# LuletterSoul/RP-Style-Transfer

Measured on NVIDIA B200. Metric: stylized images/sec @512^2 (multiscale RP-AdaIN transform), higher is better.
Workload: dtype f32

## Files before the change

### rp-style-transfer_b200/csrc/api.cu

```cuda
#include "common.cuh"
#include "tuning.cuh"

#include <string.h>

namespace rpst {

static thread_local char g_err[512] = "";

void set_error(const char* fmt, ...) {
    va_list ap;
    va_start(ap, fmt);
    vsnprintf(g_err, sizeof(g_err), fmt, ap);
    va_end(ap);
}

int cuda_fail(cudaError_t e, const char* what) {
    set_error("CUDA error %d (%s) in %s", (int)e, cudaGetErrorString(e), what);
    return RPST_ERR_CUDA;
}

int sm_count() {
    static int cached[64] = {0};
    int dev = 0;
    if (cudaGetDevice(&dev) != cudaSuccess || dev < 0 || dev >= 64) return 148;
    if (cached[dev] == 0) {
        int n = 0;
        if (cudaDeviceGetAttribute(&n, cudaDevAttrMultiProcessorCount, dev) != cudaSuccess || n <= 0) n = 148;
        cached[dev] = n;
    }
    return cached[dev];
}

Knobs g_knobs;

struct KnobSpec {
    const char* name;
    int64_t Knobs::*field;
    int64_t lo, hi;
};

static const KnobSpec kKnobs[] = {
    {"adain_lag_bytes", &Knobs::adain_lag_bytes, 0, INT64_MAX},
    {"adain_big_lag_bytes", &Knobs::adain_big_lag_bytes, 0, INT64_MAX},
    {"adain_mvn_lag_bytes", &Knobs::adain_mvn_lag_bytes, 0, INT64_MAX},
    {"adain_hints", &Knobs::adain_hints, 0, 1},
    {"adain_path", &Knobs::adain_path, 0, 1},
    {"adain_twin_apply", &Knobs::adain_twin_apply, 0, 1},
    {"adain_group_merge_min_spp", &Knobs::adain_group_merge_min_spp, 0, INT64_MAX},
    {"adain_merge_lead", &Knobs::adain_merge_lead, 0, INT64_MAX},
    {"seg_lag_bytes", &Knobs::seg_lag_bytes, 0, INT64_MAX},
    {"attn_flash", &Knobs::attn_flash, 0, 1},
    {"attn_flash_prof", &Knobs::attn_flash_prof, 0, INT64_MAX},
    {"wct_fused_cov", &Knobs::wct_fused_cov, 0, 1},
    {"wct_fused_apply", &Knobs::wct_fused_apply, 0, 1},
    {"wct_cov_tma", &Knobs::wct_cov_tma, 0, 1},
    {"wct_cov_prof", &Knobs::wct_cov_prof, 0, INT64_MAX},
    {"wct_roots_ns", &Knobs::wct_roots_ns, 0, 2},
    {"ns_dmma", &Knobs::ns_dmma, 0, 1},
    {"pw_x_tma", &Knobs::pw_x_tma, 0, 1},
};

static const KnobSpec* find_knob(const char* name) {
    for (const KnobSpec& k : kKnobs)
        if (!strcmp(name, k.name)) return &k;
    return nullptr;
}

int set_watchdog_adain(unsigned long long ns);
int set_watchdog_cov(unsigned long long ns);
int set_watchdog_flash(unsigned long long ns);
int set_watchdog_gemm(unsigned long long ns);
int set_watchdog_sanet(unsigned long long ns);
int set_watchdog_seg(unsigned long long ns);
int set_watchdog_pwconv(unsigned long long ns);

static int64_t g_watchdog_ms = 4000;

static int apply_watchdog(int64_t ms) {
    const unsigned long long ns = ms <= 0 ? 0ull : (unsigned long long)ms * 1000000ull;
    int count = 0, cur = 0;
    g_watchdog_ms = ms <= 0 ? 0 : ms;
    if (cudaGetDeviceCount(&count) != cudaSuccess || count <= 0) return RPST_OK;
    cudaGetDevice(&cur);
    int rc = 0;
    for (int d = 0; d < count; ++d) {
        if (cudaSetDevice(d) != cudaSuccess) continue;
        rc |= set_watchdog_adain(ns);
        rc |= set_watchdog_cov(ns);
        rc |= set_watchdog_flash(ns);
        rc |= set_watchdog_gemm(ns);
        rc |= set_watchdog_sanet(ns);
        rc |= set_watchdog_seg(ns);
        rc |= set_watchdog_pwconv(ns);
    }
    cudaSetDevice(cur);
    if (rc) {
        set_error("watchdog_ms: cudaMemcpyToSymbol failed");
        return RPST_ERR_CUDA;
    }
    return RPST_OK;
}

}

extern "C" int rpst_version(void) { return RPST_VERSION; }

namespace rpst { int64_t ns_flagged_total(); }

extern "C" const char* rpst_last_error(void) { return rpst::g_err; }

extern "C" int rpst_set_tuning(const char* name, int64_t value) {
    RPST_CHECK_ARG(name, "rpst_set_tuning: null knob name");
    if (!strcmp(name, "watchdog_ms")) return rpst::apply_watchdog(value);
    RPST_CHECK_ARG(strcmp(name, "wct_ns_flagged") != 0, "tuning knob 'wct_ns_flagged' is read-only");
    const rpst::KnobSpec* k = rpst::find_knob(name);
    RPST_CHECK_ARG(k, "unknown tuning knob '%s'", name);
    RPST_CHECK_ARG(value >= k->lo && value <= k->hi, "tuning knob '%s' takes %lld..%lld (got %lld)", name,
                   (long long)k->lo, (long long)k->hi, (long long)value);
    rpst::g_knobs.*k->field = value;
    return RPST_OK;
}

extern "C" int64_t rpst_get_tuning(const char* name) {
    if (!name) return -1;
    if (!strcmp(name, "watchdog_ms")) return rpst::g_watchdog_ms;
    if (!strcmp(name, "wct_ns_flagged")) return rpst::ns_flagged_total();
    const rpst::KnobSpec* k = rpst::find_knob(name);
    return k ? rpst::g_knobs.*k->field : -1;
}
```

### rp-style-transfer_b200/csrc/seg.cu

```cuda
#include "common.cuh"
#include "tuning.cuh"
#include "plane_io.cuh"
#include "async.cuh"

namespace rpst {
namespace {

constexpr int kLabels = 256;
constexpr int kNoIndex = 0x7f7f7f7f;

struct SegParams {
    const float* content;
    const float* style;
    const uint8_t* c_lab;
    const uint8_t* s_lab;
    const float* prev;
    float* out;
    const int* cmap;
    const int* smap;
    int64_t n, channels, hw_c, hw_s, out_batch_stride;
    float eps;
    int hints;
    int ipp_c, ipp_s, lag;
    unsigned total_items;
    unsigned* ticket;
    int* done;
    int* ready;
    int* cnt;
    int* first;
    float2* gsum;
    float4* coef;
    const int* run_flag;
};

__global__ void __launch_bounds__(256) seg_hist_kernel(const uint8_t* __restrict__ c_lab, const uint8_t* __restrict__ s_lab,
                                                       int64_t hw_c, int64_t hw_s, int* __restrict__ cnt,
                                                       int* __restrict__ first) {
    __shared__ int h[kLabels];
    __shared__ int f[kLabels];
    const int which = blockIdx.z;
    const int64_t n = blockIdx.y;
    const int64_t hw = which ? hw_s : hw_c;
    const uint8_t* lab = (which ? s_lab : c_lab) + n * hw;
    h[threadIdx.x] = 0;
    f[threadIdx.x] = kNoIndex;
    __syncthreads();
    const int64_t per_block = (hw + gridDim.x - 1) / gridDim.x;
    const int64_t beg = blockIdx.x * per_block;
    const int64_t end = beg + per_block < hw ? beg + per_block : hw;
    for (int64_t i = beg + threadIdx.x; i < end; i += blockDim.x) {
        int l = lab[i];
        atomicAdd(&h[l], 1);
        atomicMin(&f[l], (int)i);
    }
    __syncthreads();
    const int64_t slot = (n * 2 + which) * kLabels + threadIdx.x;
    if (h[threadIdx.x]) {
        atomicAdd(&cnt[slot], h[threadIdx.x]);
        atomicMin(&first[slot], f[threadIdx.x]);
    }
}

__device__ __forceinline__ int64_t src_plane(const int* map, int64_t plane) {
    return map ? (int64_t)__ldg(map + plane) : plane;
}

__device__ __forceinline__ bool label_usable(int nc, int ns) {
    return nc > 10 && ns > 10 && (int64_t)nc < 100ll * ns && (int64_t)ns < 100ll * nc;
}

struct SegItem {
    int kind;
    int64_t plane;
    int chunk;
};

__device__ __forceinline__ SegItem seg_decode(unsigned t, const SegParams& p) {
    const int64_t planes = p.n * p.channels;
    const int64_t st = p.ipp_c + p.ipp_s;
    const int64_t lag = p.lag < planes ? p.lag : planes;
    SegItem it;
    int64_t tt = t;
    auto stats = [&](int64_t plane, int64_t u) {
        it.plane = plane;
        if (u < p.ipp_c) { it.kind = 0; it.chunk = (int)u; }
        else { it.kind = 1; it.chunk = (int)(u - p.ipp_c); }
    };
    if (tt < lag * st) { stats(tt / st, tt % st); return it; }
    tt -= lag * st;
    const int64_t round = st + p.ipp_c;
    const int64_t steady = (planes - lag) * round;
    if (tt < steady) {
        int64_t r = tt / round, u = tt % round;
        if (u < st) stats(r + lag, u);
        else { it.kind = 2; it.plane = r; it.chunk = (int)(u - st); }
        return it;
    }
    tt -= steady;
    it.kind = 2; it.plane = (planes - lag) + tt / p.ipp_c; it.chunk = (int)(tt % p.ipp_c);
    return it;
}

template <int VEC>
__device__ __forceinline__ void load_labels(int (&lab)[VEC], const uint8_t* p) {
    if constexpr (VEC == 4) {
        uchar4 v = __ldg(reinterpret_cast<const uchar4*>(p));
        lab[0] = v.x; lab[1] = v.y; lab[2] = v.z; lab[3] = v.w;
    } else {
        lab[0] = __ldg(p);
    }
}

template <int VEC>
__global__ void __launch_bounds__(kPipeThreads, 3) seg_pipe_kernel(SegParams p) {
    constexpr int T = kPipeThreads;
    constexpr int CHUNK = T * kPerThread * VEC;
    static_assert(T == kLabels, "one thread per label value");
    __shared__ float s_shift[kLabels];
    __shared__ float s_acc[kLabels][2];
    __shared__ float4 s_coef[kLabels];
    __shared__ unsigned char s_use[kLabels];
    __shared__ unsigned s_ticket;
    __shared__ int s_last;

    const uint64_t pol_first = policy_evict_first();
    const uint64_t pol_last = policy_evict_last();
    const bool hint = p.hints != 0;
    const int lane = threadIdx.x & 31;
    if (p.run_flag != nullptr && __ldg(p.run_flag) == 0) return;

    if (threadIdx.x == 0) s_ticket = atomicAdd(p.ticket, 1u);
    __syncthreads();
    unsigned t = s_ticket;

    while (t < p.total_items) {
        unsigned next = 0;
        if (threadIdx.x == 0) next = atomicAdd(p.ticket, 1u);
        const SegItem it = seg_decode(t, p);
        const int64_t sample = it.plane / p.channels;
        const int* cnt_c = p.cnt + (sample * 2 + 0) * kLabels;
        const int* cnt_s = p.cnt + (sample * 2 + 1) * kLabels;

        if (it.kind < 2) {
            const bool is_style = it.kind == 1;
            const int64_t hw = is_style ? p.hw_s : p.hw_c;
            const float* x = is_style ? p.style + src_plane(p.smap, it.plane) * hw : p.content + src_plane(p.cmap, it.plane) * hw;
            const uint8_t* labels = (is_style ? p.s_lab : p.c_lab) + sample * hw;
            const int* first = p.first + (sample * 2 + it.kind) * kLabels;
            const int64_t e0 = (int64_t)it.chunk * CHUNK;
            const int64_t rem = hw - e0;
            const int nvec = (int)((rem < CHUNK ? rem : CHUNK) / VEC);
            {
                const int l = threadIdx.x;
                const bool use = label_usable(__ldg(cnt_c + l), __ldg(cnt_s + l));
                s_use[l] = use;
                s_shift[l] = use ? __ldg(x + __ldg(first + l)) : 0.f;
                s_acc[l][0] = 0.f;
                s_acc[l][1] = 0.f;
            }
            __syncthreads();
            int cur = -1;
            float shift = 0.f, a1 = 0.f, a2 = 0.f;
            const uint64_t xpol = is_style ? pol_first : pol_last;
#pragma unroll
            for (int b = 0; b < kBatches; ++b) {
                float v[kBatch][VEC];
                load_batch<VEC, T>(v, x + e0, b, nvec, xpol, hint);
#pragma unroll
                for (int j = 0; j < kBatch; ++j) {
                    const int idx = (b * kBatch + j) * T + threadIdx.x;
                    if (idx < nvec) {
                        int lab[VEC];
                        load_labels<VEC>(lab, labels + e0 + (int64_t)idx * VEC);
#pragma unroll
                        for (int e = 0; e < VEC; ++e) {
                            const int l = lab[e];
                            if (l != cur) {
                                if (cur >= 0) {
                                    atomicAdd(&s_acc[cur][0], a1);
                                    atomicAdd(&s_acc[cur][1], a2);
                                }
                                if (s_use[l]) { cur = l; shift = s_shift[l]; }
                                else cur = -1;
                                a1 = 0.f; a2 = 0.f;
                            }
                            if (cur >= 0) {
                                const float d = v[j][e] - shift;
                                a1 += d;
                                a2 = fmaf(d, d, a2);
                            }
                        }
                    }
                }
            }
            unsigned remaining = __ballot_sync(0xffffffffu, cur >= 0);
            while (remaining) {
                const int leader = __ffs(remaining) - 1;
                const int l = __shfl_sync(0xffffffffu, cur, leader);
                const bool mine = cur == l;
                const float r1 = warp_sum(mine ? a1 : 0.f);
                const float r2 = warp_sum(mine ? a2 : 0.f);
                if (lane == leader) {
                    atomicAdd(&s_acc[l][0], r1);
                    atomicAdd(&s_acc[l][1], r2);
                }
                remaining &= ~__ballot_sync(0xffffffffu, mine);
            }
            __syncthreads();
            {
                const int l = threadIdx.x;
                const float r1 = s_acc[l][0], r2 = s_acc[l][1];
                if (r1 != 0.f || r2 != 0.f) {
                    float2* g = p.gsum + (it.plane * 2 + it.kind) * kLabels + l;
                    atomicAdd(&g->x, r1);
                    atomicAdd(&g->y, r2);
                }
            }
            __threadfence();
            __syncthreads();
            if (threadIdx.x == 0) {
                int old = atomicAdd(&p.done[it.plane], 1);
                s_last = (old == p.ipp_c + p.ipp_s - 1);
            }
            __syncthreads();
            if (s_last) {
                __threadfence();
                const int l = threadIdx.x;
                const int nc = __ldg(cnt_c + l), ns = __ldg(cnt_s + l);
                float4 cf = make_float4(0.f, 1.f, 0.f, 0.f);
                if (label_usable(nc, ns)) {
                    const float kc = __ldg(p.content + src_plane(p.cmap, it.plane) * p.hw_c + __ldg(p.first + (sample * 2 + 0) * kLabels + l));
                    const float ks = __ldg(p.style + src_plane(p.smap, it.plane) * p.hw_s + __ldg(p.first + (sample * 2 + 1) * kLabels + l));
                    const float2 gc = __ldcg(p.gsum + (it.plane * 2 + 0) * kLabels + l);
                    const float2 gs = __ldcg(p.gsum + (it.plane * 2 + 1) * kLabels + l);
                    const float fnc = (float)nc, fns = (float)ns;
                    const float mu_c = kc + gc.x / fnc;
                    const float mu_s = ks + gs.x / fns;
                    const float m2c = fmaxf(gc.y - gc.x * gc.x / fnc, 0.f);
                    const float m2s = fmaxf(gs.y - gs.x * gs.x / fns, 0.f);
                    const float sd_c = sqrtf(m2c / (fnc - 1.f) + p.eps);
                    const float sd_s = sqrtf(m2s / (fns - 1.f) + p.eps);
                    cf = make_float4(mu_c, sd_s / sd_c, mu_s, 1.f);
                }
                __stcg(&p.coef[it.plane * kLabels + l], cf);
                __threadfence();
                __syncthreads();
                if (threadIdx.x == 0) st_release(&p.ready[it.plane], 1);
            }
        } else {
            const int64_t e0 = (int64_t)it.chunk * CHUNK;
            const int64_t rem = p.hw_c - e0;
            const int nvec = (int)((rem < CHUNK ? rem : CHUNK) / VEC);
            const float* cbase = p.content + src_plane(p.cmap, it.plane) * p.hw_c + e0;
            const float* pbase = p.prev ? p.prev + it.plane * p.hw_c + e0 : nullptr;
            float* obase = p.out + sample * p.out_batch_stride + (it.plane - sample * p.channels) * p.hw_c + e0;
            const uint8_t* labels = p.c_lab + sample * p.hw_c + e0;
            float c[kBatch][VEC], pv[kBatch][VEC];
            load_batch<VEC, T>(c, cbase, 0, nvec, pol_first, hint);
            if (pbase) load_batch<VEC, T>(pv, pbase, 0, nvec, pol_first, hint);
            if (threadIdx.x == 0) {
                while (ld_acquire(&p.ready[it.plane]) == 0) __nanosleep(100);
            }
            __syncthreads();
            s_coef[threadIdx.x] = __ldcg(&p.coef[it.plane * kLabels + threadIdx.x]);
            __syncthreads();
#pragma unroll
            for (int b = 0; b < kBatches; ++b) {
                if (b > 0) {
                    load_batch<VEC, T>(c, cbase, b, nvec, pol_first, hint);
                    if (pbase) load_batch<VEC, T>(pv, pbase, b, nvec, pol_first, hint);
                }
#pragma unroll
                for (int j = 0; j < kBatch; ++j) {
                    const int idx = (b * kBatch + j) * T + threadIdx.x;
                    if (idx < nvec) {
                        int lab[VEC];
                        load_labels<VEC>(lab, labels + (int64_t)idx * VEC);
                        float o[VEC];
#pragma unroll
                        for (int e = 0; e < VEC; ++e) {
                            const float4 cf = s_coef[lab[e]];
                            const float y = fmaf(c[j][e] - cf.x, cf.y, cf.z);
                            o[e] = pbase ? y + pv[j][e] : y;
                        }
                        store_vec<VEC>(obase + (int64_t)idx * VEC, o, pol_first, hint);
                    }
                }
            }
        }
        __syncthreads();
        if (threadIdx.x == 0) s_ticket = next;
        __syncthreads();
        t = s_ticket;
    }
}

constexpr int kSegItemElems = 4096;
constexpr int kSegPrevElems = 2048;
constexpr int kSegHalfElems = kSegPrevElems;
constexpr int kSegDataBytes = (kSegItemElems > 2 * kSegPrevElems ? kSegItemElems : 2 * kSegPrevElems) * 4;
constexpr int kSegStageBytes = kSegDataBytes + kSegItemElems;
constexpr int kSegDepth = 2;
constexpr int kSegGroups = 4;
constexpr int kSegGroupWarps = 4;
constexpr int kSegGroupThreads = kSegGroupWarps * 32;
constexpr int kSegWarpVecs = kSegItemElems / 4 / kSegGroupWarps;
constexpr int kSegLaneVecs = kSegWarpVecs / 32;
constexpr int kSegTicketBatch = 8;
constexpr int kMaxDense = 64;

struct SegTmaParams {
    const float* content;
    const float* style;
    const uint8_t* c_lab;
    const uint8_t* s_lab;
    const float* prev;
    float* out;
    const int* cmap;
    const int* smap;
    int64_t n, channels, hw_c, hw_s, out_batch_stride;
    float eps;
    int ic, is, lag;
    int ia, apply_elems;
    unsigned total_items;
    unsigned* ticket;
    int* ready;
    const int* cnt;
    const int* first;
    float* shift;
    const unsigned char* dense;
    const unsigned char* label_of;
    const int* dense_count;
    const int* overflow;
    float2* slots;
    int imax;
    float4* coef;
};

struct __align__(16) SegDesc {
    int64_t plane;
    int kind;
    int chunk;
    int nvec;
    int pad;
};

struct SegDecoded {
    int64_t plane;
    int kind, chunk;
};

__global__ void __launch_bounds__(kLabels) seg_dense_kernel(const int* __restrict__ cnt, unsigned char* __restrict__ dense,
                                                            unsigned char* __restrict__ label_of,
                                                            int* __restrict__ dense_count, int* __restrict__ overflow) {
    __shared__ int warp_cnt[kLabels / 32];
    const int sample = blockIdx.x, l = threadIdx.x, lane = l & 31, w = l >> 5;
    const bool use = label_usable(cnt[(sample * 2 + 0) * kLabels + l], cnt[(sample * 2 + 1) * kLabels + l]);
    const unsigned m = __ballot_sync(0xffffffffu, use);
    if (lane == 0) warp_cnt[w] = __popc(m);
    __syncthreads();
    int base = 0, total = 0;
    for (int i = 0; i < kLabels / 32; ++i) {
        if (i < w) base += warp_cnt[i];
        total += warp_cnt[i];
    }
    const int id = base + __popc(m & ((1u << lane) - 1u));
    dense[sample * kLabels + l] = (use && id < kMaxDense) ? (unsigned char)id : (unsigned char)255;
    if (use && id < kMaxDense) label_of[sample * kMaxDense + id] = (unsigned char)l;
    if (l == 0) {
        dense_count[sample] = total < kMaxDense ? total : kMaxDense;
        if (total > kMaxDense) atomicOr(overflow, 1);
    }
}

__global__ void seg_shift_kernel(SegTmaParams p) {
    const int64_t planes = p.n * p.channels;
    const int64_t idx = blockIdx.x * (int64_t)blockDim.x + threadIdx.x;
    if (idx >= planes * 2 * kLabels) return;
    const int l = (int)(idx % kLabels), which = (int)((idx / kLabels) & 1);
    const int64_t plane = idx / (2 * kLabels), sample = plane / p.channels;
    const int slot = (int)((sample * 2 + which) * kLabels + l);
    float v = 0.f;
    if (p.cnt[slot] > 0) {
        v = which ? p.style[src_plane(p.smap, plane) * p.hw_s + p.first[slot]]
                  : p.content[src_plane(p.cmap, plane) * p.hw_c + p.first[slot]];
    }
    p.shift[idx] = v;
}

__device__ __forceinline__ bool slot2_valid(double2 v) {
    return (unsigned)(__double_as_longlong(v.x) >> 32) != 0xffffffffu && (unsigned)(__double_as_longlong(v.y) >> 32) != 0xffffffffu;
}
__device__ __forceinline__ double2 ld_slot2(const double2* p) {
    double2 v;
    asm volatile("ld.global.cg.v2.f64 {%0,%1}, [%2];" : "=d"(v.x), "=d"(v.y) : "l"(p) : "memory");
    return v;
}
__device__ __forceinline__ float2 ld_slot1(const float2* p) {
    float2 v;
    asm volatile("ld.global.cg.v2.f32 {%0,%1}, [%2];" : "=f"(v.x), "=f"(v.y) : "l"(p) : "memory");
    return v;
}
__device__ __forceinline__ bool slot1_valid(float2 v) {
    return __float_as_uint(v.x) != 0xffffffffu && __float_as_uint(v.y) != 0xffffffffu;
}

__device__ __forceinline__ float canon_f(float v) {
    return __float_as_uint(v) == 0xffffffffu ? __uint_as_float(0x7fc00000u) : v;
}

__device__ __forceinline__ void seg_decode(unsigned t, const SegTmaParams& p, int& kind, int64_t& plane, int& chunk) {
    const unsigned P = (unsigned)(p.n * p.channels), L = (unsigned)p.lag, Lm = L - 1;
    const unsigned Ic = (unsigned)p.ic, St = (unsigned)(p.ic + p.is), Ia = (unsigned)p.ia;
    auto stat = [&](unsigned pl, unsigned u) {
        plane = pl;
        if (u < Ic) { kind = 0; chunk = (int)u; } else { kind = 1; chunk = (int)(u - Ic); }
    };
    unsigned n = (L - Lm) * St;
    if (t < n) { stat(t / St, t % St); return; }
    t -= n; n = Lm * (St + 1);
    if (t < n) {
        const unsigned j = t / (St + 1), u = t % (St + 1);
        if (u < St) stat((L - Lm) + j, u); else { kind = 3; plane = j; chunk = 0; }
        return;
    }
    t -= n; n = (P - L) * (St + 1 + Ia);
    if (t < n) {
        const unsigned j = t / (St + 1 + Ia), u = t % (St + 1 + Ia);
        if (u < St) stat(L + j, u);
        else if (u == St) { kind = 3; plane = Lm + j; chunk = 0; }
        else { kind = 2; plane = j; chunk = (int)(u - St - 1); }
        return;
    }
    t -= n; n = (L - Lm) * (1 + Ia);
    if (t < n) {
        const unsigned j = t / (1 + Ia), u = t % (1 + Ia);
        if (u == 0) { kind = 3; plane = (P - L + Lm) + j; chunk = 0; }
        else { kind = 2; plane = (P - L) + j; chunk = (int)(u - 1); }
        return;
    }
    t -= n;
    kind = 2; plane = (P - Lm) + t / Ia; chunk = (int)(t % Ia);
}

constexpr int kSegCoefBytes = (kMaxDense + 2) * 16;
constexpr int kSegCacheBytes = (kSegCoefBytes + kLabels * 4 + kLabels + 2 * kMaxDense * 2 * 4 +
                                kSegGroupWarps * 32 * 16 + 2 * kSegGroupWarps * 32 * 2 * 4 + 127) / 128 * 128;
constexpr int kSegMergeThreads = 64;
constexpr int kSegMailbox = 8;

__device__ __forceinline__ void seg_warp_totals(float2* tab, int lane, int cur, float a1, float a2) {
    const int key = cur >= 0 ? cur : -1;
    const unsigned peers = __match_any_sync(0xffffffffu, key);
    const int steps = (int)__reduce_max_sync(0xffffffffu, (unsigned)__popc(peers));
    float s1 = a1, s2 = a2;
    unsigned rem = peers & (peers - 1u);
    const bool leader = (peers & ((1u << lane) - 1u)) == 0u;
    for (int k = 1; k < steps; ++k) {
        const int src = rem ? __ffs(rem) - 1 : lane;
        const float x1 = __shfl_sync(0xffffffffu, a1, src), x2 = __shfl_sync(0xffffffffu, a2, src);
        if (rem) { s1 += x1; s2 += x2; }
        rem &= rem - 1u;
    }
    tab[lane] = make_float2(0.f, 0.f);
    __syncwarp();
    if (leader && key >= 0) tab[key] = make_float2(s1, s2);
    __syncwarp();
}

__global__ void __launch_bounds__(32 + kSegGroups * kSegGroupThreads + kSegMergeThreads, 1) seg_tma_kernel(SegTmaParams p) {
    constexpr int S = kSegGroups * kSegDepth;
    constexpr int STAGE_BYTES = kSegStageBytes;
    constexpr int CACHE_BYTES = kSegCacheBytes;
    extern __shared__ __align__(128) unsigned char smem_raw[];
    unsigned char* stages = smem_raw;
    unsigned char* caches = smem_raw + (size_t)S * STAGE_BYTES;
    SegDesc* desc = reinterpret_cast<SegDesc*>(caches + (size_t)kSegGroups * ((CACHE_BYTES + 127) / 128 * 128));
    uint64_t* full = reinterpret_cast<uint64_t*>(desc + S);
    uint64_t* empty = full + S;
    uint64_t* mfull = empty + S;
    uint64_t* mempty = mfull + kSegMailbox;
    int64_t* mbox = reinterpret_cast<int64_t*>(mempty + kSegMailbox);
    SegDecoded* dec = reinterpret_cast<SegDecoded*>(mbox + kSegMailbox);

    const int warp = threadIdx.x >> 5, lane = threadIdx.x & 31;
    if (__ldg(p.overflow) != 0) return;
    if (threadIdx.x == 0) {
        for (int s = 0; s < S; ++s) {
            mbar_init(&full[s], 1);
            mbar_init(&empty[s], kSegGroupWarps);
        }
        for (int s = 0; s < kSegMailbox; ++s) {
            mbar_init(&mfull[s], 1);
            mbar_init(&mempty[s], kSegMergeThreads / 32);
        }
        mbar_fence_init();
    }
    __syncthreads();

    if (warp == 0) {
        const uint64_t pol_first = policy_evict_first();
        const uint64_t pol_last = policy_evict_last();
        unsigned next_base = 0;
        if (lane == 0) next_base = atomicAdd(p.ticket, (unsigned)kSegTicketBatch) + 1u;
        unsigned seq = 0, mseq = 0;
        for (;;) {
            const unsigned base = __shfl_sync(0xffffffffu, next_base, 0);
            if (lane == 0) next_base = atomicAdd(p.ticket, (unsigned)kSegTicketBatch) + 1u;
            static_assert(kSegGroups * kSegDepth >= kSegTicketBatch, "a batch must not reuse a stage");
            int kind = 3, chunk = 0;
            int64_t plane = 0, splane = 0;
            if (lane < kSegTicketBatch) {
                kind = -1;
                const unsigned t = base + (unsigned)lane;
                if (t < p.total_items) seg_decode(t, p, kind, plane, chunk);
                dec[lane].kind = kind; dec[lane].chunk = chunk; dec[lane].plane = plane;
                if (kind == 1) splane = src_plane(p.smap, plane);
                else if (kind == 0 || kind == 2) splane = src_plane(p.cmap, plane);
            }
            __syncwarp();
            const unsigned stopmask = __ballot_sync(0xffffffffu, kind < 0);
            const int nvalid = stopmask ? __ffs(stopmask) - 1 : kSegTicketBatch;
            if (lane == 0) {
                for (int i = 0; i < nvalid; ++i) {
                    if (dec[i].kind == 3) {
                        const int ms = (int)(mseq % kSegMailbox);
                        mbar_wait_quiet(&mempty[ms], ((mseq / kSegMailbox) & 1u) ^ 1u);
                        mbox[ms] = dec[i].plane;
                        mbar_arrive(&mfull[ms]);
                        ++mseq;
                    }
                }
            }
            const bool is_item = lane < nvalid && kind != 3;
            const unsigned itemmask = __ballot_sync(0xffffffffu, is_item);
            const int my_pos = __popc(itemmask & ((1u << lane) - 1u));
            if (is_item) {
                const unsigned my_seq = seq + (unsigned)my_pos;
                const unsigned k = my_seq / kSegGroups;
                const int stage = (int)(my_seq % kSegGroups) * kSegDepth + (int)(k % kSegDepth);
                mbar_wait_quiet(&empty[stage], ((k / kSegDepth) & 1u) ^ 1u);
                SegDesc* d = &desc[stage];
                d->plane = plane; d->kind = kind; d->chunk = chunk;
                const bool is_style = kind == 1;
                const int64_t hw = is_style ? p.hw_s : p.hw_c;
                const int item_elems = kind == 2 ? p.apply_elems : kSegItemElems;
                const int64_t e0 = (int64_t)chunk * item_elems;
                const int64_t rem = hw - e0;
                const int nvec = (int)((rem < item_elems ? rem : item_elems) / 4);
                d->nvec = nvec;
                const uint32_t bytes = (uint32_t)nvec * 16u;
                unsigned char* st = stages + (size_t)stage * STAGE_BYTES;
                const int64_t sample = (int)plane / (int)p.channels;
                const float* src = (is_style ? p.style : p.content) + splane * hw + e0;
                const uint8_t* lab = (is_style ? p.s_lab : p.c_lab) + sample * hw + e0;
                const bool has_prev = kind == 2 && p.prev != nullptr;
                mbar_arrive_expect_tx(&full[stage], bytes + (has_prev ? bytes : 0u) + (uint32_t)nvec * 4u);
                tma_load_1d(st, src, bytes, &full[stage], kind == 0 ? pol_last : pol_first);
                if (has_prev)
                    tma_load_1d(st + kSegHalfElems * 4, p.prev + plane * hw + e0, bytes, &full[stage], pol_first);
                tma_load_1d(st + kSegDataBytes, lab, (uint32_t)nvec * 4u, &full[stage], pol_last);
            }
            __syncwarp();
            seq += (unsigned)__popc(itemmask);
            bool finished = false;
            if (stopmask != 0u) {
                if (lane == 0) {
                    for (int g = 0; g < kSegGroups; ++g, ++seq) {
                        const unsigned k = seq / kSegGroups;
                        const int stage = (int)(seq % kSegGroups) * kSegDepth + (int)(k % kSegDepth);
                        mbar_wait_quiet(&empty[stage], ((k / kSegDepth) & 1u) ^ 1u);
                        desc[stage].kind = -1;
                        mbar_arrive(&full[stage]);
                    }
                    const int ms = (int)(mseq % kSegMailbox);
                    mbar_wait_quiet(&mempty[ms], ((mseq / kSegMailbox) & 1u) ^ 1u);
                    mbox[ms] = -1;
                    mbar_arrive(&mfull[ms]);
                }
                finished = true;
            }
            if (finished) return;
            __syncwarp();
        }
    }

    if (warp > kSegGroups * kSegGroupWarps) {
        __shared__ double s_merge[kSegMergeThreads][4];
        const int t = threadIdx.x - (32 + kSegGroups * kSegGroupThreads);
        for (unsigned mseq = 0;; ++mseq) {
            const int ms = (int)(mseq % kSegMailbox);
            mbar_wait_quiet(&mfull[ms], (mseq / kSegMailbox) & 1u, 64);
            const int64_t plane = mbox[ms];
            __syncwarp();
            if (lane == 0) mbar_arrive(&mempty[ms]);
            if (plane < 0) break;
            const int64_t sample = plane / p.channels;
            const int dcount = __ldg(p.dense_count + sample);
            const int parts = dcount > 0 ? kSegMergeThreads / dcount : 1;
            const int dn = dcount > 0 ? t % dcount : 0;
            const int part = dcount > 0 ? t / dcount : parts;
            double s4[4] = {0.0, 0.0, 0.0, 0.0};
            if (part < parts) {
#pragma unroll
                for (int which = 0; which < 2; ++which) {
                    const int items = which ? p.is : p.ic;
                    const int per = (items + parts - 1) / parts;
                    const int lo = part * per, hi = min(items, lo + per);
                    const float2* base = p.slots + ((plane * 2 + which) * p.imax) * kMaxDense + dn;
                    constexpr int kUnroll = 32;
                    for (int c0 = lo; c0 < hi; c0 += kUnroll) {
                        float2 v[kUnroll];
#pragma unroll
                        for (int u = 0; u < kUnroll; ++u) {
                            v[u] = make_float2(0.f, 0.f);
                            if (c0 + u < hi) v[u] = ld_slot1(base + (int64_t)(c0 + u) * kMaxDense);
                        }
#pragma unroll
                        for (int u = 0; u < kUnroll; ++u) {
                            if (c0 + u < hi) {
                                if (!slot1_valid(v[u])) {
                                    const float2* sp = base + (int64_t)(c0 + u) * kMaxDense;
                                    const uint64_t t0 = global_timer_ns();
                                    do {
                                        __nanosleep(64);
                                        v[u] = ld_slot1(sp);
                                        if (watchdog_expired(t0)) __trap();
                                    } while (!slot1_valid(v[u]));
                                }
                                s4[which * 2 + 0] += (double)v[u].x;
                                s4[which * 2 + 1] += (double)v[u].y;
                            }
                        }
                    }
                }
            }
#pragma unroll
            for (int q = 0; q < 4; ++q) s_merge[t][q] = s4[q];
            named_bar_sync(15, kSegMergeThreads);
            if (t < dcount) {
                for (int q = 1; q < parts; ++q) {
#pragma unroll
                    for (int e = 0; e < 4; ++e) s4[e] += s_merge[q * dcount + t][e];
                }
                const int l = __ldg(p.label_of + sample * kMaxDense + dn);
                const double dnc = (double)__ldg(p.cnt + (sample * 2 + 0) * kLabels + l);
                const double dns = (double)__ldg(p.cnt + (sample * 2 + 1) * kLabels + l);
                const double kc = (double)__ldg(p.shift + (plane * 2 + 0) * kLabels + l);
                const double ks = (double)__ldg(p.shift + (plane * 2 + 1) * kLabels + l);
                const double mu_c = kc + s4[0] / dnc, mu_s = ks + s4[2] / dns;
                const double m2c = fmax(s4[1] - s4[0] * s4[0] / dnc, 0.0), m2s = fmax(s4[3] - s4[2] * s4[2] / dns, 0.0);
                const double sd_c = sqrt(m2c / (dnc - 1.0) + (double)p.eps), sd_s = sqrt(m2s / (dns - 1.0) + (double)p.eps);
                __stcg(&p.coef[plane * kLabels + l], make_float4((float)mu_c, (float)(sd_s / sd_c), (float)mu_s, 1.f));
            }
            for (int l = t; l < kLabels; l += kSegMergeThreads)
                if (__ldg(p.dense + sample * kLabels + l) == 255) __stcg(&p.coef[plane * kLabels + l], make_float4(0.f, 1.f, 0.f, 0.f));
            __threadfence();
            named_bar_sync(15, kSegMergeThreads);
            if (t == 0) st_release(&p.ready[plane], 1);
        }
        return;
    }

    const int group = (warp - 1) / kSegGroupWarps;
    const int gw = (warp - 1) % kSegGroupWarps;
    const int gt = gw * 32 + lane;
    unsigned char* cache = caches + (size_t)group * ((CACHE_BYTES + 127) / 128 * 128);
    float4* c_coef = reinterpret_cast<float4*>(cache);
    float* c_shift = reinterpret_cast<float*>(cache + kSegCoefBytes);
    unsigned char* c_dense = cache + kSegCoefBytes + kLabels * 4;
    float* c_acc = reinterpret_cast<float*>(c_dense + kLabels);
    float4* c_stage = reinterpret_cast<float4*>(c_acc + 2 * kMaxDense * 2);
    float* c_wtot = reinterpret_cast<float*>(c_stage + kSegGroupWarps * 32);
    const uint64_t pol_first = policy_evict_first();
    int64_t cached_stat = -1;
    int64_t cached_apply = -1;
    int64_t cached_sample = -1;
    int dcount = 0;
    unsigned sparity = 0;
    for (int i = gt; i < 2 * kMaxDense * 2; i += kSegGroupThreads) c_acc[i] = 0.f;
    named_bar_sync(1 + group, kSegGroupThreads);

    for (unsigned seq = group;; seq += kSegGroups) {
        const unsigned k = seq / kSegGroups;
        const int stage = group * kSegDepth + (int)(k % kSegDepth);
        mbar_wait_quiet(&full[stage], (k / kSegDepth) & 1u);
        const SegDesc* d = &desc[stage];
        const int kind = d->kind;
        if (kind < 0) break;
        const int64_t plane = d->plane;
        const int chunk = d->chunk;
        const int warp_vecs = (kind == 2 ? p.apply_elems : kSegItemElems) / 4 / kSegGroupWarps;
        const int wvec = min(max(d->nvec - gw * warp_vecs, 0), warp_vecs);
        const int64_t sample = (int)plane / (int)p.channels;
        unsigned char* st = stages + (size_t)stage * STAGE_BYTES;
        const float4* a4 = reinterpret_cast<const float4*>(st) + gw * warp_vecs;
        const float4* b4 = reinterpret_cast<const float4*>(st + kSegHalfElems * 4) + gw * warp_vecs;
        const uint32_t* l4 = reinterpret_cast<const uint32_t*>(st + kSegDataBytes) + gw * warp_vecs;

        {
            if (sample != cached_sample) {
                named_bar_sync(1 + group, kSegGroupThreads);
                for (int l = gt; l < kLabels; l += kSegGroupThreads) c_dense[l] = __ldg(p.dense + sample * kLabels + l);
                dcount = __ldg(p.dense_count + sample);
                named_bar_sync(1 + group, kSegGroupThreads);
                cached_sample = sample;
            }
        }

        if (kind <= 1) {
            const int64_t key = plane * 2 + kind;
            if (key != cached_stat) {
                named_bar_sync(1 + group, kSegGroupThreads);
                for (int l = gt; l < kLabels; l += kSegGroupThreads) c_shift[l] = __ldg(p.shift + key * kLabels + l);
                named_bar_sync(1 + group, kSegGroupThreads);
                cached_stat = key;
            }
            float* acc = c_acc + sparity * (kMaxDense * 2);
            int cur = -1;
            uint32_t cur4 = 0xffffffffu;
            float shift = 0.f, a1 = 0.f, a2 = 0.f;
            float4 vv[kSegLaneVecs];
            uint32_t lww[kSegLaneVecs];
#pragma unroll
            for (int j = 0; j < kSegLaneVecs; ++j) {
                const int idx = lane * kSegLaneVecs + ((j + lane) & (kSegLaneVecs - 1));
                if (idx < wvec) { vv[j] = a4[idx]; lww[j] = l4[idx]; }
            }
            __syncwarp();
            if (lane == 0) mbar_arrive(&empty[stage]);
#pragma unroll
            for (int j = 0; j < kSegLaneVecs; ++j) {
                const int idx = lane * kSegLaneVecs + ((j + lane) & (kSegLaneVecs - 1));
                if (idx < wvec) {
                    const float4 v = vv[j];
                    const uint32_t lw = lww[j];
                    if (lw == cur4 && cur >= 0) {
                        const float d0 = v.x - shift, d1 = v.y - shift, d2 = v.z - shift, d3 = v.w - shift;
                        a1 += (d0 + d1) + (d2 + d3);
                        a2 = fmaf(d0, d0, a2); a2 = fmaf(d1, d1, a2); a2 = fmaf(d2, d2, a2); a2 = fmaf(d3, d3, a2);
                    } else {
                        const float e[4] = {v.x, v.y, v.z, v.w};
                        int curl = cur >= 0 ? (int)(cur4 & 0xffu) : -1;
#pragma unroll
                        for (int q = 0; q < 4; ++q) {
                            const int l = (int)((lw >> (8 * q)) & 0xffu);
                            if (l != curl) {
                                if (cur >= 0) {
                                    atomicAdd(&acc[cur * 2 + 0], a1);
                                    atomicAdd(&acc[cur * 2 + 1], a2);
                                }
                                const int dn = c_dense[l];
                                curl = l;
                                if (dn != 255) { cur = dn; shift = c_shift[l]; cur4 = (uint32_t)l * 0x01010101u; }
                                else { cur = -1; cur4 = 0xffffffffu; }
                                a1 = 0.f; a2 = 0.f;
                            }
                            if (cur >= 0) {
                                const float dd = e[q] - shift;
                                a1 += dd;
                                a2 = fmaf(dd, dd, a2);
                            }
                        }
                    }
                }
            }
            const bool staged = dcount <= 32;
            float* wt = c_wtot + (sparity * kSegGroupWarps + gw) * 64;
            if (staged) {
                seg_warp_totals(reinterpret_cast<float2*>(wt), lane, cur, a1, a2);
            } else if (cur >= 0) {
                atomicAdd(&acc[cur * 2 + 0], a1);
                atomicAdd(&acc[cur * 2 + 1], a2);
            }
            named_bar_sync(1 + group, kSegGroupThreads);
            if (gt < dcount) {
                float t1 = acc[gt * 2 + 0], t2 = acc[gt * 2 + 1];
                if (staged) {
                    const float* w0 = c_wtot + sparity * kSegGroupWarps * 64;
#pragma unroll
                    for (int q = 0; q < kSegGroupWarps; ++q) { t1 += w0[q * 64 + gt * 2 + 0]; t2 += w0[q * 64 + gt * 2 + 1]; }
                }
                const float s1 = canon_f(t1), s2 = canon_f(t2);
                acc[gt * 2 + 0] = 0.f;
                acc[gt * 2 + 1] = 0.f;
                float2* slot = p.slots + ((key * p.imax + chunk) * kMaxDense + gt);
                asm volatile("st.global.cg.v2.f32 [%0], {%1,%2};" :: "l"(slot), "f"(s1), "f"(s2) : "memory");
            }
            sparity ^= 1u;
        } else if (kind == 2) {
            if (plane != cached_apply) {
                if (lane == 0 && ld_acquire(&p.ready[plane]) == 0) {
                    const uint64_t t0 = global_timer_ns();
                    while (ld_acquire(&p.ready[plane]) == 0) {
                        __nanosleep(64);
                        if (watchdog_expired(t0)) __trap();
                    }
                }
                named_bar_sync(1 + group, kSegGroupThreads);
                if (gt < dcount) c_coef[gt] = __ldcg(&p.coef[plane * kLabels + __ldg(p.label_of + sample * kMaxDense + gt)]);
                if (gt == kSegGroupThreads - 1) c_coef[kMaxDense] = make_float4(0.f, 1.f, 0.f, 0.f);
                named_bar_sync(1 + group, kSegGroupThreads);
                cached_apply = plane;
            }
            const bool has_prev = p.prev != nullptr;
            float4* o4 = reinterpret_cast<float4*>(p.out + sample * p.out_batch_stride + (plane - sample * p.channels) * p.hw_c +
                                                   (int64_t)chunk * p.apply_elems) + gw * warp_vecs;
            uint32_t last_w = 0;
            float4 cf = c_coef[kMaxDense];
            bool have = false;
            auto coef_of = [&](uint32_t l) -> float4 { const int dn = c_dense[l]; return c_coef[dn < kMaxDense ? dn : kMaxDense]; };
#pragma unroll 8
            for (int j = 0; j < kSegLaneVecs; ++j) {
                const int idx = j * 32 + lane;
                if (idx < wvec) {
                    const float4 v = a4[idx];
                    const uint32_t lw = l4[idx];
                    float4 o;
                    const uint32_t b0 = lw & 0xffu;
                    if (lw == b0 * 0x01010101u) {
                        if (!have || lw != last_w) { cf = coef_of(b0); last_w = lw; have = true; }
                        o.x = fmaf(v.x - cf.x, cf.y, cf.z);
                        o.y = fmaf(v.y - cf.x, cf.y, cf.z);
                        o.z = fmaf(v.z - cf.x, cf.y, cf.z);
                        o.w = fmaf(v.w - cf.x, cf.y, cf.z);
                    } else {
                        const float4 c0 = coef_of(b0), c1 = coef_of((lw >> 8) & 0xffu), c2 = coef_of((lw >> 16) & 0xffu),
                                     c3 = coef_of(lw >> 24);
                        o.x = fmaf(v.x - c0.x, c0.y, c0.z);
                        o.y = fmaf(v.y - c1.x, c1.y, c1.z);
                        o.z = fmaf(v.z - c2.x, c2.y, c2.z);
                        o.w = fmaf(v.w - c3.x, c3.y, c3.z);
                    }
                    if (has_prev) {
                        const float4 q = b4[idx];
                        o.x += q.x; o.y += q.y; o.z += q.z; o.w += q.w;
                    }
                    stg_f4_hint(reinterpret_cast<float*>(o4 + idx), o, pol_first);
                }
            }
            __syncwarp();
            if (lane == 0) mbar_arrive(&empty[stage]);
        }
    }
}

__global__ void seg_export_info_kernel(const int* __restrict__ cnt, int32_t* __restrict__ info, int64_t n) {
    const int64_t i = blockIdx.x * (int64_t)blockDim.x + threadIdx.x;
    if (i >= n * kLabels) return;
    const int64_t s = i / kLabels, l = i % kLabels;
    const int nc = cnt[(s * 2 + 0) * kLabels + l], ns = cnt[(s * 2 + 1) * kLabels + l];
    info[i * 3 + 0] = nc;
    info[i * 3 + 1] = ns;
    info[i * 3 + 2] = label_usable(nc, ns) ? 1 : 0;
}

struct SegLayout {
    size_t zero_bytes;
    size_t first_off, first_bytes, coef_off, total;
    size_t done_off, cnt_off, gsum_off;
};

SegLayout seg_layout(int64_t n, int64_t c) {
    const size_t planes = (size_t)(n * c);
    SegLayout l;
    l.done_off = 256;
    l.cnt_off = align_up(l.done_off + planes * 2 * sizeof(int), 256);
    l.gsum_off = align_up(l.cnt_off + (size_t)n * 2 * kLabels * sizeof(int), 256);
    l.zero_bytes = align_up(l.gsum_off + planes * 2 * kLabels * sizeof(float2), 256);
    l.first_off = l.zero_bytes;
    l.first_bytes = align_up((size_t)n * 2 * kLabels * sizeof(int), 256);
    l.coef_off = l.first_off + l.first_bytes;
    l.total = align_up(l.coef_off + planes * kLabels * sizeof(float4), 256);
    return l;
}

inline bool aligned(const void* p, size_t a) { return (reinterpret_cast<uintptr_t>(p) & (a - 1)) == 0; }

struct SegTmaLayout {
    size_t ticket, zero_beg, ready, cnt, dcount, overflow, zero_end, first, first_bytes, shift, dense, label_of, coef,
        slots, slots_bytes, total;
};
SegTmaLayout seg_tma_layout(int64_t n, int64_t c, int64_t hw_c, int64_t hw_s) {
    const size_t planes = (size_t)(n * c);
    const size_t ic = (size_t)((hw_c + kSegItemElems - 1) / kSegItemElems), is = (size_t)((hw_s + kSegItemElems - 1) / kSegItemElems);
    const size_t imax = ic > is ? ic : is;
    SegTmaLayout l;
    size_t o = 0;
    auto take = [&](size_t bytes) { size_t at = o; o += align_up(bytes, 256); return at; };
    l.ticket = take(256);
    l.zero_beg = o;
    l.ready = take(planes * sizeof(int));
    l.cnt = take((size_t)n * 2 * kLabels * sizeof(int));
    l.dcount = take((size_t)n * sizeof(int));
    l.overflow = take(sizeof(int));
    l.zero_end = o;
    l.first_bytes = align_up((size_t)n * 2 * kLabels * sizeof(int), 256);
    l.first = take(l.first_bytes);
    l.shift = take(planes * 2 * kLabels * sizeof(float));
    l.dense = take((size_t)n * kLabels);
    l.label_of = take((size_t)n * kMaxDense);
    l.coef = take(planes * kLabels * sizeof(float4));
    l.slots_bytes = planes * 2 * imax * kMaxDense * sizeof(float2);
    l.slots = take(l.slots_bytes);
    l.total = o;
    return l;
}

int launch_seg_tma(const SegTmaParams& p, cudaStream_t st) {
    constexpr size_t stage = kSegStageBytes;
    constexpr size_t cache = kSegCacheBytes;
    constexpr size_t smem = kSegGroups * (kSegDepth * stage + cache) + kSegGroups * kSegDepth * sizeof(SegDesc) +
                            2 * kSegGroups * kSegDepth * sizeof(uint64_t) + 2 * kSegMailbox * sizeof(uint64_t) +
                            kSegMailbox * sizeof(int64_t) +
                            kSegTicketBatch * sizeof(SegDecoded);
    static PerDeviceFlag configured_on;
    bool& configured = configured_on.get();
    if (!configured) {
        RPST_CUDA(cudaFuncSetAttribute(seg_tma_kernel, cudaFuncAttributeMaxDynamicSharedMemorySize, (int)smem));
        configured = true;
    }
    int64_t grid = sm_count();
    if (grid > (int64_t)p.total_items) grid = p.total_items;
    seg_tma_kernel<<<(int)grid, 32 + kSegGroups * kSegGroupThreads + kSegMergeThreads, smem, st>>>(p);
    RPST_CUDA(cudaGetLastError());
    return RPST_OK;
}

}
}

namespace rpst {
namespace {
int64_t seg_plan_schedule(SegTmaParams& q, bool has_prev) {
    const int64_t planes = q.n * q.channels;
    q.ic = (int)((q.hw_c + kSegItemElems - 1) / kSegItemElems);
    q.is = (int)((q.hw_s + kSegItemElems - 1) / kSegItemElems);
    q.imax = q.ic > q.is ? q.ic : q.is;
    q.apply_elems = has_prev ? kSegPrevElems : kSegItemElems;
    q.ia = (int)((q.hw_c + q.apply_elems - 1) / q.apply_elems);
    const int64_t plane_bytes = q.hw_c * (int64_t)sizeof(float);
    int64_t lag = (g_knobs.seg_lag_bytes + plane_bytes - 1) / plane_bytes;
    if (lag < 3) lag = 3;
    q.lag = (int)(lag < planes ? lag : planes);
    return planes * ((int64_t)q.ic + q.is + 1 + q.ia);
}

__global__ void seg_schedule_dump_kernel(SegTmaParams p, int32_t* out) {
    const unsigned t = blockIdx.x * blockDim.x + threadIdx.x;
    if (t >= p.total_items) return;
    int kind = -1, chunk = 0;
    int64_t plane = 0;
    seg_decode(t, p, kind, plane, chunk);
    out[3 * (size_t)t + 0] = kind;
    out[3 * (size_t)t + 1] = (int32_t)plane;
    out[3 * (size_t)t + 2] = chunk;
}
}
}

using namespace rpst;

#ifdef RPST_DEBUG_EXPORTS
extern "C" int rpst_debug_seg_schedule(int64_t n, int64_t c, int64_t hw_c, int64_t hw_s, int has_prev, int32_t* tickets,
                                       int64_t max_tickets, int64_t* info, void* stream) {
    RPST_CHECK_ARG(n > 0 && c > 0 && hw_c > 0 && hw_s > 0 && info != nullptr, "debug_seg_schedule: bad arguments");
    SegTmaParams q{};
    q.n = n; q.channels = c; q.hw_c = hw_c; q.hw_s = hw_s;
    const int64_t total = seg_plan_schedule(q, has_prev != 0);
    RPST_CHECK_ARG(total < (1ll << 31), "debug_seg_schedule: too many tickets");
    q.total_items = (unsigned)total;
    info[0] = total; info[1] = q.ic; info[2] = q.is; info[3] = q.ia; info[4] = q.lag;
    if (tickets != nullptr) {
        RPST_CHECK_ARG(max_tickets >= total, "debug_seg_schedule: ticket buffer too small");
        seg_schedule_dump_kernel<<<(unsigned)((total + 255) / 256), 256, 0, static_cast<cudaStream_t>(stream)>>>(q, tickets);
        RPST_CUDA(cudaGetLastError());
    }
    return RPST_OK;
}
#endif

extern "C" size_t rpst_seg_adain_workspace_bytes(int64_t n, int64_t c, int64_t hw_c, int64_t hw_s) {
    if (n <= 0 || c <= 0) return 256;
    return seg_layout(n, c).total + seg_tma_layout(n, c, hw_c, hw_s).total;

}

namespace {
int seg_adain_fwd_impl(const float* content, const float* style, const uint8_t* c_labels, const uint8_t* s_labels,
                       const float* prev, float* out, int64_t n, int64_t c, int64_t hw_c, int64_t hw_s,
                       int64_t out_batch_stride, float eps, const int* content_map, const int* style_map,
                       int32_t* label_info, void* workspace, size_t workspace_bytes, void* stream);
}

extern "C" int rpst_seg_adain_fwd(const float* content, const float* style, const uint8_t* c_labels,
                                  const uint8_t* s_labels, const float* prev, float* out, int64_t n, int64_t c,
                                  int64_t hw_c, int64_t hw_s, float eps, int32_t* label_info, void* workspace,
                                  size_t workspace_bytes, void* stream) {
    return seg_adain_fwd_impl(content, style, c_labels, s_labels, prev, out, n, c, hw_c, hw_s, c * hw_c, eps, nullptr,
                              nullptr, label_info, workspace, workspace_bytes, stream);
}

extern "C" int rpst_seg_adain_fwd_mapped(const float* content, const float* style, const uint8_t* c_labels,
                                         const uint8_t* s_labels, const float* prev, float* out, int64_t n, int64_t c,
                                         int64_t hw_c, int64_t hw_s, int64_t out_batch_stride, float eps,
                                         const int32_t* content_map, const int32_t* style_map, int32_t* label_info,
                                         void* workspace, size_t workspace_bytes, void* stream) {
    RPST_CHECK_ARG(n * c < (1ll << 31), "seg_adain_mapped: plane index does not fit int32");
    return seg_adain_fwd_impl(content, style, c_labels, s_labels, prev, out, n, c, hw_c, hw_s, out_batch_stride, eps,
                              content_map, style_map, label_info, workspace, workspace_bytes, stream);
}

namespace {
int seg_adain_fwd_impl(const float* content, const float* style, const uint8_t* c_labels, const uint8_t* s_labels,
                       const float* prev, float* out, int64_t n, int64_t c, int64_t hw_c, int64_t hw_s,
                       int64_t out_batch_stride, float eps, const int* content_map, const int* style_map,
                       int32_t* label_info, void* workspace, size_t workspace_bytes, void* stream) {
    RPST_CHECK_ARG(n >= 0 && c >= 0 && hw_c >= 0 && hw_s >= 0, "seg_adain: negative size");
    if (n == 0 || c == 0 || hw_c == 0) return RPST_OK;
    RPST_CHECK_ARG(content && style && c_labels && s_labels && out, "seg_adain: null pointer");
    RPST_CHECK_ARG(hw_s > 0, "seg_adain: empty style map");
    RPST_CHECK_ARG(hw_c < (1ll << 31) && hw_s < (1ll << 31), "seg_adain: plane too large");
    RPST_CHECK_ARG(out_batch_stride >= c * hw_c, "seg_adain: out_batch_stride (%lld) < c*hw_c (%lld)",
                   (long long)out_batch_stride, (long long)(c * hw_c));
    RPST_CHECK_ARG(out != content && out != style && out != prev, "seg_adain: out must not alias an input");
    const size_t need = rpst_seg_adain_workspace_bytes(n, c, hw_c, hw_s);
    if (workspace == nullptr || workspace_bytes < need) {
        set_error("seg_adain: workspace too small (%zu < %zu bytes)", workspace_bytes, need);
        return RPST_ERR_WORKSPACE;
    }
    RPST_CHECK_ARG(aligned(workspace, 256), "seg_adain: workspace must be 256-byte aligned");
    cudaStream_t st = static_cast<cudaStream_t>(stream);
    char* base = static_cast<char*>(workspace);
    const int64_t hw_max0 = hw_c > hw_s ? hw_c : hw_s;
    int hist_blocks0 = (int)((hw_max0 + 16383) / 16384);
    if (hist_blocks0 > 256) hist_blocks0 = 256;
    const bool tma_ok = g_knobs.adain_path == 0 && hw_c % 16 == 0 && hw_s % 16 == 0 &&
                        aligned(content, 16) && aligned(style, 16) && aligned(out, 16) && out_batch_stride % 4 == 0 &&
                        (!prev || aligned(prev, 16)) && aligned(c_labels, 16) && aligned(s_labels, 16);
    const int* run_flag = nullptr;
    if (tma_ok) {
        const SegTmaLayout t = seg_tma_layout(n, c, hw_c, hw_s);
        SegTmaParams q{};
        q.content = content; q.style = style; q.c_lab = c_labels; q.s_lab = s_labels; q.prev = prev; q.out = out;
        q.cmap = content_map; q.smap = style_map;
        q.n = n; q.channels = c; q.hw_c = hw_c; q.hw_s = hw_s; q.out_batch_stride = out_batch_stride; q.eps = eps;
        q.ticket = reinterpret_cast<unsigned*>(base + t.ticket);
        q.ready = reinterpret_cast<int*>(base + t.ready);
        int* cnt = reinterpret_cast<int*>(base + t.cnt);
        int* first = reinterpret_cast<int*>(base + t.first);
        int* dcount = reinterpret_cast<int*>(base + t.dcount);
        int* overflow = reinterpret_cast<int*>(base + t.overflow);
        unsigned char* dense = reinterpret_cast<unsigned char*>(base + t.dense);
        unsigned char* label_of = reinterpret_cast<unsigned char*>(base + t.label_of);
        q.cnt = cnt; q.first = first; q.dense = dense; q.label_of = label_of; q.dense_count = dcount; q.overflow = overflow;
        q.shift = reinterpret_cast<float*>(base + t.shift);
        q.coef = reinterpret_cast<float4*>(base + t.coef);
        q.slots = reinterpret_cast<float2*>(base + t.slots);
        RPST_CUDA(cudaMemsetAsync(base + t.ticket, 0xff, 256, st));
        RPST_CUDA(cudaMemsetAsync(base + t.zero_beg, 0, t.zero_end - t.zero_beg, st));
        RPST_CUDA(cudaMemsetAsync(base + t.first, 0x7f, t.first_bytes, st));
        RPST_CUDA(cudaMemsetAsync(base + t.slots, 0xff, t.slots_bytes, st));
        seg_hist_kernel<<<dim3(hist_blocks0, (unsigned)n, 2), 256, 0, st>>>(c_labels, s_labels, hw_c, hw_s, cnt, first);
        RPST_CUDA(cudaGetLastError());
        seg_dense_kernel<<<(unsigned)n, kLabels, 0, st>>>(cnt, dense, label_of, dcount, overflow);
        RPST_CUDA(cudaGetLastError());
        if (label_info) {
            const int64_t tot = n * kLabels;
            seg_export_info_kernel<<<(unsigned)((tot + 255) / 256), 256, 0, st>>>(cnt, label_info, n);
            RPST_CUDA(cudaGetLastError());
            label_info = nullptr;
        }
        const int64_t planes = n * c;
        seg_shift_kernel<<<(unsigned)((planes * 2 * kLabels + 255) / 256), 256, 0, st>>>(q);
        RPST_CUDA(cudaGetLastError());
        const int64_t total = seg_plan_schedule(q, prev != nullptr);
        RPST_CHECK_ARG(total < (1ll << 31), "seg_adain: too many work items (%lld); split the call", (long long)total);
        q.total_items = (unsigned)total;
        const int rc = launch_seg_tma(q, st);
        if (rc) return rc;
        run_flag = overflow;
        base += t.total;
    }
    const SegLayout l = seg_layout(n, c);
    SegParams p{};
    p.content = content; p.style = style; p.c_lab = c_labels; p.s_lab = s_labels; p.prev = prev; p.out = out;
    p.cmap = content_map; p.smap = style_map;
    p.n = n; p.channels = c; p.hw_c = hw_c; p.hw_s = hw_s; p.out_batch_stride = out_batch_stride; p.eps = eps;
    p.hints = (int)g_knobs.adain_hints;
    p.ticket = reinterpret_cast<unsigned*>(base);
    p.done = reinterpret_cast<int*>(base + l.done_off);
    p.ready = p.done + n * c;
    p.cnt = reinterpret_cast<int*>(base + l.cnt_off);
    p.gsum = reinterpret_cast<float2*>(base + l.gsum_off);
    p.first = reinterpret_cast<int*>(base + l.first_off);
    p.coef = reinterpret_cast<float4*>(base + l.coef_off);
    p.run_flag = run_flag;
    RPST_CUDA(cudaMemsetAsync(base, 0, l.zero_bytes, st));
    RPST_CUDA(cudaMemsetAsync(base + l.first_off, 0x7f, l.first_bytes, st));

    const int64_t hw_max = hw_c > hw_s ? hw_c : hw_s;
    int hist_blocks = (int)((hw_max + 16383) / 16384);
    if (hist_blocks > 256) hist_blocks = 256;
    seg_hist_kernel<<<dim3(hist_blocks, (unsigned)n, 2), 256, 0, st>>>(c_labels, s_labels, hw_c, hw_s, p.cnt, p.first);
    RPST_CUDA(cudaGetLastError());
    if (label_info) {
        const int64_t tot = n * kLabels;
        seg_export_info_kernel<<<(unsigned)((tot + 255) / 256), 256, 0, st>>>(p.cnt, label_info, n);
        RPST_CUDA(cudaGetLastError());
    }

    const bool vec = hw_c % 4 == 0 && hw_s % 4 == 0 && aligned(content, 16) && aligned(style, 16) && aligned(out, 16) &&
                     out_batch_stride % 4 == 0 && (!prev || aligned(prev, 16)) && aligned(c_labels, 4) && aligned(s_labels, 4);
    const int64_t chunk = (int64_t)kPipeThreads * kPerThread * (vec ? 4 : 1);
    p.ipp_c = (int)((hw_c + chunk - 1) / chunk);
    p.ipp_s = (int)((hw_s + chunk - 1) / chunk);
    const int64_t plane_bytes = hw_c * (int64_t)sizeof(float);
    int64_t lag = (g_knobs.adain_lag_bytes + plane_bytes - 1) / plane_bytes;
    if (lag < 3) lag = 3;
    const int64_t planes = n * c;
    p.lag = (int)(lag < planes ? lag : planes);
    const int64_t total = planes * (2ll * p.ipp_c + p.ipp_s);
    RPST_CHECK_ARG(total < (1ll << 31), "seg_adain: too many work items (%lld); split the call", (long long)total);
    p.total_items = (unsigned)total;
    int64_t grid = (int64_t)sm_count() * 3;
    if (grid > total) grid = total;
    if (vec) seg_pipe_kernel<4><<<(int)grid, kPipeThreads, 0, st>>>(p);
    else seg_pipe_kernel<1><<<(int)grid, kPipeThreads, 0, st>>>(p);
    RPST_CUDA(cudaGetLastError());
    return RPST_OK;
}
}

RPST_WATCHDOG_SETTER(seg)
```

### rp-style-transfer_b200/csrc/tuning.cuh

```cuda
#pragma once
#include <stdint.h>

namespace rpst {

struct Knobs {
    int64_t adain_lag_bytes = 32ll << 20;
    int64_t adain_big_lag_bytes = 128ll << 20;
    int64_t adain_mvn_lag_bytes = 44ll << 20;
    int64_t adain_hints = 1;
    int64_t adain_path = 0;
    int64_t adain_twin_apply = 1;
    int64_t adain_group_merge_min_spp = 512;
    int64_t adain_merge_lead = 0;
    int64_t seg_lag_bytes = 256ll << 20;
    int64_t attn_flash = 1;
    int64_t attn_flash_prof = 0;
    int64_t wct_fused_cov = 1;
    int64_t wct_fused_apply = 1;
    int64_t wct_cov_tma = 1;
    int64_t wct_cov_prof = 0;
    int64_t wct_roots_ns = 1;
    int64_t ns_dmma = 1;
    int64_t pw_x_tma = 1;
};

extern Knobs g_knobs;

}
```

Baseline: 3478.

## Split persistent segmented AdaIN kernel into stats, merge and apply launches

Replaces the single persistent warp-specialized TMA kernel, which used a ticket scheduler, lagged per-plane merge mailboxes and per-item slot buffers, with three ordinary launches: a multi-CTA stats kernel that writes per-row double partials, a per-plane merge kernel, and an apply kernel. This removes the ticket atomics, spin-waits and slot memsets, and lets more stats CTAs reside per SM. In exchange it loses the overlap between statistics and apply work, adds launch boundaries, and re-reads content planes from memory in the apply pass. The lag knob is replaced by a rows-per-CTA knob.

```diff
diff --git a/rp-style-transfer_b200/csrc/api.cu b/rp-style-transfer_b200/csrc/api.cu
--- a/rp-style-transfer_b200/csrc/api.cu
+++ b/rp-style-transfer_b200/csrc/api.cu
@@ -48,7 +48,7 @@
     {"adain_twin_apply", &Knobs::adain_twin_apply, 0, 1},
     {"adain_group_merge_min_spp", &Knobs::adain_group_merge_min_spp, 0, INT64_MAX},
     {"adain_merge_lead", &Knobs::adain_merge_lead, 0, INT64_MAX},
-    {"seg_lag_bytes", &Knobs::seg_lag_bytes, 0, INT64_MAX},
+    {"seg_stats_items", &Knobs::seg_stats_items, 1, 1024},
     {"attn_flash", &Knobs::attn_flash, 0, 1},
     {"attn_flash_prof", &Knobs::attn_flash_prof, 0, INT64_MAX},
     {"wct_fused_cov", &Knobs::wct_fused_cov, 0, 1},
diff --git a/rp-style-transfer_b200/csrc/seg.cu b/rp-style-transfer_b200/csrc/seg.cu
--- a/rp-style-transfer_b200/csrc/seg.cu
+++ b/rp-style-transfer_b200/csrc/seg.cu
@@ -297,16 +297,15 @@
 
 constexpr int kSegItemElems = 4096;
 constexpr int kSegPrevElems = 2048;
-constexpr int kSegHalfElems = kSegPrevElems;
-constexpr int kSegDataBytes = (kSegItemElems > 2 * kSegPrevElems ? kSegItemElems : 2 * kSegPrevElems) * 4;
-constexpr int kSegStageBytes = kSegDataBytes + kSegItemElems;
-constexpr int kSegDepth = 2;
-constexpr int kSegGroups = 4;
+constexpr int kSegStageBytes = kSegItemElems * 4 + kSegItemElems;
+constexpr int kSegStages = 2;
+constexpr int kSegStatsCtas = 5;
 constexpr int kSegGroupWarps = 4;
 constexpr int kSegGroupThreads = kSegGroupWarps * 32;
 constexpr int kSegWarpVecs = kSegItemElems / 4 / kSegGroupWarps;
 constexpr int kSegLaneVecs = kSegWarpVecs / 32;
-constexpr int kSegTicketBatch = 8;
+constexpr int kSegApplyThreads = 256;
+constexpr int kSegApplyChunks = 8;
 constexpr int kMaxDense = 64;
 
 struct SegTmaParams {
@@ -320,11 +319,10 @@
     const int* smap;
     int64_t n, channels, hw_c, hw_s, out_batch_stride;
     float eps;
-    int ic, is, lag;
+    int ic, is;
     int ia, apply_elems;
-    unsigned total_items;
-    unsigned* ticket;
-    int* ready;
+    int row_items;
+    int rc, rs;
     const int* cnt;
     const int* first;
     float* shift;
@@ -332,22 +330,8 @@
     const unsigned char* label_of;
     const int* dense_count;
     const int* overflow;
-    float2* slots;
-    int imax;
+    double2* rows;
     float4* coef;
-};
-
-struct __align__(16) SegDesc {
-    int64_t plane;
-    int kind;
-    int chunk;
-    int nvec;
-    int pad;
-};
-
-struct SegDecoded {
-    int64_t plane;
-    int kind, chunk;
 };
 
 __global__ void __launch_bounds__(kLabels) seg_dense_kernel(const int* __restrict__ cnt, unsigned char* __restrict__ dense,
@@ -388,67 +372,6 @@
     p.shift[idx] = v;
 }
 
-__device__ __forceinline__ bool slot2_valid(double2 v) {
-    return (unsigned)(__double_as_longlong(v.x) >> 32) != 0xffffffffu && (unsigned)(__double_as_longlong(v.y) >> 32) != 0xffffffffu;
-}
-__device__ __forceinline__ double2 ld_slot2(const double2* p) {
-    double2 v;
-    asm volatile("ld.global.cg.v2.f64 {%0,%1}, [%2];" : "=d"(v.x), "=d"(v.y) : "l"(p) : "memory");
-    return v;
-}
-__device__ __forceinline__ float2 ld_slot1(const float2* p) {
-    float2 v;
-    asm volatile("ld.global.cg.v2.f32 {%0,%1}, [%2];" : "=f"(v.x), "=f"(v.y) : "l"(p) : "memory");
-    return v;
-}
-__device__ __forceinline__ bool slot1_valid(float2 v) {
-    return __float_as_uint(v.x) != 0xffffffffu && __float_as_uint(v.y) != 0xffffffffu;
-}
-
-__device__ __forceinline__ float canon_f(float v) {
-    return __float_as_uint(v) == 0xffffffffu ? __uint_as_float(0x7fc00000u) : v;
-}
-
-__device__ __forceinline__ void seg_decode(unsigned t, const SegTmaParams& p, int& kind, int64_t& plane, int& chunk) {
-    const unsigned P = (unsigned)(p.n * p.channels), L = (unsigned)p.lag, Lm = L - 1;
-    const unsigned Ic = (unsigned)p.ic, St = (unsigned)(p.ic + p.is), Ia = (unsigned)p.ia;
-    auto stat = [&](unsigned pl, unsigned u) {
-        plane = pl;
-        if (u < Ic) { kind = 0; chunk = (int)u; } else { kind = 1; chunk = (int)(u - Ic); }
-    };
-    unsigned n = (L - Lm) * St;
-    if (t < n) { stat(t / St, t % St); return; }
-    t -= n; n = Lm * (St + 1);
-    if (t < n) {
-        const unsigned j = t / (St + 1), u = t % (St + 1);
-        if (u < St) stat((L - Lm) + j, u); else { kind = 3; plane = j; chunk = 0; }
-        return;
-    }
-    t -= n; n = (P - L) * (St + 1 + Ia);
-    if (t < n) {
-        const unsigned j = t / (St + 1 + Ia), u = t % (St + 1 + Ia);
-        if (u < St) stat(L + j, u);
-        else if (u == St) { kind = 3; plane = Lm + j; chunk = 0; }
-        else { kind = 2; plane = j; chunk = (int)(u - St - 1); }
-        return;
-    }
-    t -= n; n = (L - Lm) * (1 + Ia);
-    if (t < n) {
-        const unsigned j = t / (1 + Ia), u = t % (1 + Ia);
-        if (u == 0) { kind = 3; plane = (P - L + Lm) + j; chunk = 0; }
-        else { kind = 2; plane = (P - L) + j; chunk = (int)(u - 1); }
-        return;
-    }
-    t -= n;
-    kind = 2; plane = (P - Lm) + t / Ia; chunk = (int)(t % Ia);
-}
-
-constexpr int kSegCoefBytes = (kMaxDense + 2) * 16;
-constexpr int kSegCacheBytes = (kSegCoefBytes + kLabels * 4 + kLabels + 2 * kMaxDense * 2 * 4 +
-                                kSegGroupWarps * 32 * 16 + 2 * kSegGroupWarps * 32 * 2 * 4 + 127) / 128 * 128;
-constexpr int kSegMergeThreads = 64;
-constexpr int kSegMailbox = 8;
-
 __device__ __forceinline__ void seg_warp_totals(float2* tab, int lane, int cur, float a1, float a2) {
     const int key = cur >= 0 ? cur : -1;
     const unsigned peers = __match_any_sync(0xffffffffu, key);
@@ -468,379 +391,235 @@
     __syncwarp();
 }
 
-__global__ void __launch_bounds__(32 + kSegGroups * kSegGroupThreads + kSegMergeThreads, 1) seg_tma_kernel(SegTmaParams p) {
-    constexpr int S = kSegGroups * kSegDepth;
-    constexpr int STAGE_BYTES = kSegStageBytes;
-    constexpr int CACHE_BYTES = kSegCacheBytes;
-    extern __shared__ __align__(128) unsigned char smem_raw[];
-    unsigned char* stages = smem_raw;
-    unsigned char* caches = smem_raw + (size_t)S * STAGE_BYTES;
-    SegDesc* desc = reinterpret_cast<SegDesc*>(caches + (size_t)kSegGroups * ((CACHE_BYTES + 127) / 128 * 128));
-    uint64_t* full = reinterpret_cast<uint64_t*>(desc + S);
-    uint64_t* empty = full + S;
-    uint64_t* mfull = empty + S;
-    uint64_t* mempty = mfull + kSegMailbox;
-    int64_t* mbox = reinterpret_cast<int64_t*>(mempty + kSegMailbox);
-    SegDecoded* dec = reinterpret_cast<SegDecoded*>(mbox + kSegMailbox);
-
+template <class Release>
+__device__ __forceinline__ void seg_item_stats(const float4* a4, const uint32_t* l4, int wvec, int lane,
+                                               const unsigned char* c_dense, const float* c_shift, float* acc,
+                                               float* wt, bool staged, Release release) {
+    int cur = -1;
+    uint32_t cur4 = 0xffffffffu;
+    float shift = 0.f, a1 = 0.f, a2 = 0.f;
+    float4 vv[kSegLaneVecs];
+    uint32_t lww[kSegLaneVecs];
+#pragma unroll
+    for (int j = 0; j < kSegLaneVecs; ++j) {
+        const int idx = lane * kSegLaneVecs + ((j + lane) & (kSegLaneVecs - 1));
+        if (idx < wvec) { vv[j] = a4[idx]; lww[j] = l4[idx]; }
+    }
+#pragma unroll
+    for (int j = 0; j < kSegLaneVecs; ++j) {
+        const int idx = lane * kSegLaneVecs + ((j + lane) & (kSegLaneVecs - 1));
+        if (idx < wvec) {
+            const float4 v = vv[j];
+            const uint32_t lw = lww[j];
+            if (lw == cur4 && cur >= 0) {
+                const float d0 = v.x - shift, d1 = v.y - shift, d2 = v.z - shift, d3 = v.w - shift;
+                a1 += (d0 + d1) + (d2 + d3);
+                a2 = fmaf(d0, d0, a2); a2 = fmaf(d1, d1, a2); a2 = fmaf(d2, d2, a2); a2 = fmaf(d3, d3, a2);
+            } else {
+                const float e[4] = {v.x, v.y, v.z, v.w};
+                int curl = cur >= 0 ? (int)(cur4 & 0xffu) : -1;
+#pragma unroll
+                for (int q = 0; q < 4; ++q) {
+                    const int l = (int)((lw >> (8 * q)) & 0xffu);
+                    if (l != curl) {
+                        if (cur >= 0) {
+                            atomicAdd(&acc[cur * 2 + 0], a1);
+                            atomicAdd(&acc[cur * 2 + 1], a2);
+                        }
+                        const int dn = c_dense[l];
+                        curl = l;
+                        if (dn != 255) { cur = dn; shift = c_shift[l]; cur4 = (uint32_t)l * 0x01010101u; }
+                        else { cur = -1; cur4 = 0xffffffffu; }
+                        a1 = 0.f; a2 = 0.f;
+                    }
+                    if (cur >= 0) {
+                        const float dd = e[q] - shift;
+                        a1 += dd;
+                        a2 = fmaf(dd, dd, a2);
+                    }
+                }
+            }
+        }
+    }
+    release();
+    if (staged) {
+        seg_warp_totals(reinterpret_cast<float2*>(wt), lane, cur, a1, a2);
+    } else if (cur >= 0) {
+        atomicAdd(&acc[cur * 2 + 0], a1);
+        atomicAdd(&acc[cur * 2 + 1], a2);
+    }
+}
+
+__global__ void __launch_bounds__(32 + kSegGroupThreads, kSegStatsCtas) seg_stats_kernel(SegTmaParams p) {
+    __shared__ __align__(128) unsigned char stages[kSegStages][kSegStageBytes];
+    __shared__ uint64_t full[kSegStages], empty[kSegStages];
+    __shared__ float c_shift[kLabels];
+    __shared__ unsigned char c_dense[kLabels];
+    __shared__ float c_acc[2][kMaxDense * 2];
+    __shared__ float c_wtot[2][kSegGroupWarps * 64];
+    if (__ldg(p.overflow) != 0) return;
+
+    const int rows = p.rc + p.rs;
+    const int64_t plane = blockIdx.x / rows;
+    const int row = (int)(blockIdx.x % rows);
+    const int which = row < p.rc ? 0 : 1;
+    const int i0 = (which ? row - p.rc : row) * p.row_items;
+    const int count = min(p.row_items, (which ? p.is : p.ic) - i0);
+    const int64_t sample = plane / p.channels;
+    const int64_t hw = which ? p.hw_s : p.hw_c;
     const int warp = threadIdx.x >> 5, lane = threadIdx.x & 31;
-    if (__ldg(p.overflow) != 0) return;
     if (threadIdx.x == 0) {
-        for (int s = 0; s < S; ++s) {
+        for (int s = 0; s < kSegStages; ++s) {
             mbar_init(&full[s], 1);
             mbar_init(&empty[s], kSegGroupWarps);
         }
-        for (int s = 0; s < kSegMailbox; ++s) {
-            mbar_init(&mfull[s], 1);
-            mbar_init(&mempty[s], kSegMergeThreads / 32);
-        }
         mbar_fence_init();
     }
+    for (int l = threadIdx.x; l < kLabels; l += blockDim.x) {
+        c_shift[l] = __ldg(p.shift + (plane * 2 + which) * kLabels + l);
+        c_dense[l] = __ldg(p.dense + sample * kLabels + l);
+    }
+    for (int i = threadIdx.x; i < 2 * kMaxDense * 2; i += blockDim.x) (&c_acc[0][0])[i] = 0.f;
     __syncthreads();
 
     if (warp == 0) {
-        const uint64_t pol_first = policy_evict_first();
-        const uint64_t pol_last = policy_evict_last();
-        unsigned next_base = 0;
-        if (lane == 0) next_base = atomicAdd(p.ticket, (unsigned)kSegTicketBatch) + 1u;
-        unsigned seq = 0, mseq = 0;
-        for (;;) {
-            const unsigned base = __shfl_sync(0xffffffffu, next_base, 0);
-            if (lane == 0) next_base = atomicAdd(p.ticket, (unsigned)kSegTicketBatch) + 1u;
-            static_assert(kSegGroups * kSegDepth >= kSegTicketBatch, "a batch must not reuse a stage");
-            int kind = 3, chunk = 0;
-            int64_t plane = 0, splane = 0;
-            if (lane < kSegTicketBatch) {
-                kind = -1;
-                const unsigned t = base + (unsigned)lane;
-                if (t < p.total_items) seg_decode(t, p, kind, plane, chunk);
-                dec[lane].kind = kind; dec[lane].chunk = chunk; dec[lane].plane = plane;
-                if (kind == 1) splane = src_plane(p.smap, plane);
-                else if (kind == 0 || kind == 2) splane = src_plane(p.cmap, plane);
-            }
-            __syncwarp();
-            const unsigned stopmask = __ballot_sync(0xffffffffu, kind < 0);
-            const int nvalid = stopmask ? __ffs(stopmask) - 1 : kSegTicketBatch;
-            if (lane == 0) {
-                for (int i = 0; i < nvalid; ++i) {
-                    if (dec[i].kind == 3) {
-                        const int ms = (int)(mseq % kSegMailbox);
-                        mbar_wait_quiet(&mempty[ms], ((mseq / kSegMailbox) & 1u) ^ 1u);
-                        mbox[ms] = dec[i].plane;
-                        mbar_arrive(&mfull[ms]);
-                        ++mseq;
-                    }
-                }
-            }
-            const bool is_item = lane < nvalid && kind != 3;
-            const unsigned itemmask = __ballot_sync(0xffffffffu, is_item);
-            const int my_pos = __popc(itemmask & ((1u << lane) - 1u));
-            if (is_item) {
-                const unsigned my_seq = seq + (unsigned)my_pos;
-                const unsigned k = my_seq / kSegGroups;
-                const int stage = (int)(my_seq % kSegGroups) * kSegDepth + (int)(k % kSegDepth);
-                mbar_wait_quiet(&empty[stage], ((k / kSegDepth) & 1u) ^ 1u);
-                SegDesc* d = &desc[stage];
-                d->plane = plane; d->kind = kind; d->chunk = chunk;
-                const bool is_style = kind == 1;
-                const int64_t hw = is_style ? p.hw_s : p.hw_c;
-                const int item_elems = kind == 2 ? p.apply_elems : kSegItemElems;
-                const int64_t e0 = (int64_t)chunk * item_elems;
-                const int64_t rem = hw - e0;
-                const int nvec = (int)((rem < item_elems ? rem : item_elems) / 4);
-                d->nvec = nvec;
-                const uint32_t bytes = (uint32_t)nvec * 16u;
-                unsigned char* st = stages + (size_t)stage * STAGE_BYTES;
-                const int64_t sample = (int)plane / (int)p.channels;
-                const float* src = (is_style ? p.style : p.content) + splane * hw + e0;
-                const uint8_t* lab = (is_style ? p.s_lab : p.c_lab) + sample * hw + e0;
-                const bool has_prev = kind == 2 && p.prev != nullptr;
-                mbar_arrive_expect_tx(&full[stage], bytes + (has_prev ? bytes : 0u) + (uint32_t)nvec * 4u);
-                tma_load_1d(st, src, bytes, &full[stage], kind == 0 ? pol_last : pol_first);
-                if (has_prev)
-                    tma_load_1d(st + kSegHalfElems * 4, p.prev + plane * hw + e0, bytes, &full[stage], pol_first);
-                tma_load_1d(st + kSegDataBytes, lab, (uint32_t)nvec * 4u, &full[stage], pol_last);
-            }
-            __syncwarp();
-            seq += (unsigned)__popc(itemmask);
-            bool finished = false;
-            if (stopmask != 0u) {
-                if (lane == 0) {
-                    for (int g = 0; g < kSegGroups; ++g, ++seq) {
-                        const unsigned k = seq / kSegGroups;
-                        const int stage = (int)(seq % kSegGroups) * kSegDepth + (int)(k % kSegDepth);
-                        mbar_wait_quiet(&empty[stage], ((k / kSegDepth) & 1u) ^ 1u);
-                        desc[stage].kind = -1;
-                        mbar_arrive(&full[stage]);
-                    }
-                    const int ms = (int)(mseq % kSegMailbox);
-                    mbar_wait_quiet(&mempty[ms], ((mseq / kSegMailbox) & 1u) ^ 1u);
-                    mbox[ms] = -1;
-                    mbar_arrive(&mfull[ms]);
-                }
-                finished = true;
-            }
-            if (finished) return;
-            __syncwarp();
-        }
-    }
-
-    if (warp > kSegGroups * kSegGroupWarps) {
-        __shared__ double s_merge[kSegMergeThreads][4];
-        const int t = threadIdx.x - (32 + kSegGroups * kSegGroupThreads);
-        for (unsigned mseq = 0;; ++mseq) {
-            const int ms = (int)(mseq % kSegMailbox);
-            mbar_wait_quiet(&mfull[ms], (mseq / kSegMailbox) & 1u, 64);
-            const int64_t plane = mbox[ms];
-            __syncwarp();
-            if (lane == 0) mbar_arrive(&mempty[ms]);
-            if (plane < 0) break;
-            const int64_t sample = plane / p.channels;
-            const int dcount = __ldg(p.dense_count + sample);
-            const int parts = dcount > 0 ? kSegMergeThreads / dcount : 1;
-            const int dn = dcount > 0 ? t % dcount : 0;
-            const int part = dcount > 0 ? t / dcount : parts;
-            double s4[4] = {0.0, 0.0, 0.0, 0.0};
-            if (part < parts) {
-#pragma unroll
-                for (int which = 0; which < 2; ++which) {
-                    const int items = which ? p.is : p.ic;
-                    const int per = (items + parts - 1) / parts;
-                    const int lo = part * per, hi = min(items, lo + per);
-                    const float2* base = p.slots + ((plane * 2 + which) * p.imax) * kMaxDense + dn;
-                    constexpr int kUnroll = 32;
-                    for (int c0 = lo; c0 < hi; c0 += kUnroll) {
-                        float2 v[kUnroll];
-#pragma unroll
-                        for (int u = 0; u < kUnroll; ++u) {
-                            v[u] = make_float2(0.f, 0.f);
-                            if (c0 + u < hi) v[u] = ld_slot1(base + (int64_t)(c0 + u) * kMaxDense);
-                        }
-#pragma unroll
-                        for (int u = 0; u < kUnroll; ++u) {
-                            if (c0 + u < hi) {
-                                if (!slot1_valid(v[u])) {
-                                    const float2* sp = base + (int64_t)(c0 + u) * kMaxDense;
-                                    const uint64_t t0 = global_timer_ns();
-                                    do {
-                                        __nanosleep(64);
-                                        v[u] = ld_slot1(sp);
-                                        if (watchdog_expired(t0)) __trap();
-                                    } while (!slot1_valid(v[u]));
-                                }
-                                s4[which * 2 + 0] += (double)v[u].x;
-                                s4[which * 2 + 1] += (double)v[u].y;
-                            }
-                        }
-                    }
-                }
-            }
-#pragma unroll
-            for (int q = 0; q < 4; ++q) s_merge[t][q] = s4[q];
-            named_bar_sync(15, kSegMergeThreads);
-            if (t < dcount) {
-                for (int q = 1; q < parts; ++q) {
-#pragma unroll
-                    for (int e = 0; e < 4; ++e) s4[e] += s_merge[q * dcount + t][e];
-                }
-                const int l = __ldg(p.label_of + sample * kMaxDense + dn);
-                const double dnc = (double)__ldg(p.cnt + (sample * 2 + 0) * kLabels + l);
-                const double dns = (double)__ldg(p.cnt + (sample * 2 + 1) * kLabels + l);
-                const double kc = (double)__ldg(p.shift + (plane * 2 + 0) * kLabels + l);
-                const double ks = (double)__ldg(p.shift + (plane * 2 + 1) * kLabels + l);
-                const double mu_c = kc + s4[0] / dnc, mu_s = ks + s4[2] / dns;
-                const double m2c = fmax(s4[1] - s4[0] * s4[0] / dnc, 0.0), m2s = fmax(s4[3] - s4[2] * s4[2] / dns, 0.0);
-                const double sd_c = sqrt(m2c / (dnc - 1.0) + (double)p.eps), sd_s = sqrt(m2s / (dns - 1.0) + (double)p.eps);
-                __stcg(&p.coef[plane * kLabels + l], make_float4((float)mu_c, (float)(sd_s / sd_c), (float)mu_s, 1.f));
-            }
-            for (int l = t; l < kLabels; l += kSegMergeThreads)
-                if (__ldg(p.dense + sample * kLabels + l) == 255) __stcg(&p.coef[plane * kLabels + l], make_float4(0.f, 1.f, 0.f, 0.f));
-            __threadfence();
-            named_bar_sync(15, kSegMergeThreads);
-            if (t == 0) st_release(&p.ready[plane], 1);
+        if (lane == 0) {
+            const float* src = which ? p.style + src_plane(p.smap, plane) * hw : p.content + src_plane(p.cmap, plane) * hw;
+            const uint8_t* lab = (which ? p.s_lab : p.c_lab) + sample * hw;
+            const uint64_t pol_first = policy_evict_first();
+            const uint64_t pol_last = policy_evict_last();
+            for (int k = 0; k < count; ++k) {
+                const int s = k % kSegStages;
+                mbar_wait_quiet(&empty[s], ((k / kSegStages) & 1u) ^ 1u);
+                fence_proxy_async_smem();
+                const int64_t e0 = (int64_t)(i0 + k) * kSegItemElems;
+                const uint32_t elems = (uint32_t)min(hw - e0, (int64_t)kSegItemElems);
+                mbar_arrive_expect_tx(&full[s], elems * 5u);
+                tma_load_1d(stages[s], src + e0, elems * 4u, &full[s], pol_first);
+                tma_load_1d(stages[s] + kSegItemElems * 4, lab + e0, elems, &full[s], pol_last);
+            }
         }
         return;
     }
 
-    const int group = (warp - 1) / kSegGroupWarps;
-    const int gw = (warp - 1) % kSegGroupWarps;
-    const int gt = gw * 32 + lane;
-    unsigned char* cache = caches + (size_t)group * ((CACHE_BYTES + 127) / 128 * 128);
-    float4* c_coef = reinterpret_cast<float4*>(cache);
-    float* c_shift = reinterpret_cast<float*>(cache + kSegCoefBytes);
-    unsigned char* c_dense = cache + kSegCoefBytes + kLabels * 4;
-    float* c_acc = reinterpret_cast<float*>(c_dense + kLabels);
-    float4* c_stage = reinterpret_cast<float4*>(c_acc + 2 * kMaxDense * 2);
-    float* c_wtot = reinterpret_cast<float*>(c_stage + kSegGroupWarps * 32);
+    const int gw = warp - 1, gt = threadIdx.x - 32;
+    const int dcount = __ldg(p.dense_count + sample);
+    const bool staged = dcount <= 32;
+    double s1 = 0.0, s2 = 0.0;
+    for (int k = 0; k < count; ++k) {
+        const int s = k % kSegStages, par = k & 1;
+        mbar_wait_quiet(&full[s], (k / kSegStages) & 1u);
+        const int nvec = (int)(min(hw - (int64_t)(i0 + k) * kSegItemElems, (int64_t)kSegItemElems) / 4);
+        const int wvec = min(max(nvec - gw * kSegWarpVecs, 0), kSegWarpVecs);
+        const float4* a4 = reinterpret_cast<const float4*>(stages[s]) + gw * kSegWarpVecs;
+        const uint32_t* l4 = reinterpret_cast<const uint32_t*>(stages[s] + kSegItemElems * 4) + gw * kSegWarpVecs;
+        seg_item_stats(a4, l4, wvec, lane, c_dense, c_shift, c_acc[par], c_wtot[par] + gw * 64, staged, [&] {
+            __syncwarp();
+            if (lane == 0) mbar_arrive(&empty[s]);
+        });
+        named_bar_sync(1, kSegGroupThreads);
+        if (gt < dcount) {
+            float t1 = c_acc[par][gt * 2 + 0], t2 = c_acc[par][gt * 2 + 1];
+            if (staged) {
+#pragma unroll
+                for (int q = 0; q < kSegGroupWarps; ++q) { t1 += c_wtot[par][q * 64 + gt * 2 + 0]; t2 += c_wtot[par][q * 64 + gt * 2 + 1]; }
+            }
+            c_acc[par][gt * 2 + 0] = 0.f;
+            c_acc[par][gt * 2 + 1] = 0.f;
+            s1 += (double)t1;
+            s2 += (double)t2;
+        }
+    }
+    if (gt < dcount) p.rows[((int64_t)blockIdx.x * kMaxDense) + gt] = make_double2(s1, s2);
+}
+
+__global__ void seg_merge_kernel(SegTmaParams p) {
+    if (__ldg(p.overflow) != 0) return;
+    const int64_t plane = blockIdx.x, sample = plane / p.channels;
+    const int t = threadIdx.x;
+    const int dcount = __ldg(p.dense_count + sample);
+    if (t < dcount) {
+        const double2* r = p.rows + plane * (p.rc + p.rs) * kMaxDense + t;
+        double s4[4] = {0.0, 0.0, 0.0, 0.0};
+#pragma unroll 4
+        for (int i = 0; i < p.rc; ++i) {
+            const double2 v = r[(int64_t)i * kMaxDense];
+            s4[0] += v.x; s4[1] += v.y;
+        }
+        r += (int64_t)p.rc * kMaxDense;
+#pragma unroll 4
+        for (int i = 0; i < p.rs; ++i) {
+            const double2 v = r[(int64_t)i * kMaxDense];
+            s4[2] += v.x; s4[3] += v.y;
+        }
+        const int l = __ldg(p.label_of + sample * kMaxDense + t);
+        const double dnc = (double)__ldg(p.cnt + (sample * 2 + 0) * kLabels + l);
+        const double dns = (double)__ldg(p.cnt + (sample * 2 + 1) * kLabels + l);
+        const double kc = (double)__ldg(p.shift + (plane * 2 + 0) * kLabels + l);
+        const double ks = (double)__ldg(p.shift + (plane * 2 + 1) * kLabels + l);
+        const double mu_c = kc + s4[0] / dnc, mu_s = ks + s4[2] / dns;
+        const double m2c = fmax(s4[1] - s4[0] * s4[0] / dnc, 0.0), m2s = fmax(s4[3] - s4[2] * s4[2] / dns, 0.0);
+        const double sd_c = sqrt(m2c / (dnc - 1.0) + (double)p.eps), sd_s = sqrt(m2s / (dns - 1.0) + (double)p.eps);
+        p.coef[plane * kLabels + l] = make_float4((float)mu_c, (float)(sd_s / sd_c), (float)mu_s, 1.f);
+    }
+    for (int l = t; l < kLabels; l += kMaxDense)
+        if (__ldg(p.dense + sample * kLabels + l) == 255) p.coef[plane * kLabels + l] = make_float4(0.f, 1.f, 0.f, 0.f);
+}
+
+template <bool PREV>
+__global__ void __launch_bounds__(kSegApplyThreads) seg_apply_kernel(SegTmaParams p) {
+    constexpr int U = (PREV ? kSegPrevElems : kSegItemElems) / 4 / kSegApplyThreads;
+    static_assert(U * 4 * kSegApplyThreads == (PREV ? kSegPrevElems : kSegItemElems), "a chunk is U float4 per thread");
+    static_assert(kSegApplyThreads == kLabels, "one coefficient per thread");
+    __shared__ float4 s_coef[kLabels];
+    if (__ldg(p.overflow) != 0) return;
+    const int per = (p.ia + kSegApplyChunks - 1) / kSegApplyChunks;
+    const int64_t plane = blockIdx.x / per;
+    const int c0 = (int)(blockIdx.x % per) * kSegApplyChunks, c1 = min(c0 + kSegApplyChunks, p.ia);
+    const int64_t sample = plane / p.channels;
+    s_coef[threadIdx.x] = p.coef[plane * kLabels + threadIdx.x];
+    __syncthreads();
     const uint64_t pol_first = policy_evict_first();
-    int64_t cached_stat = -1;
-    int64_t cached_apply = -1;
-    int64_t cached_sample = -1;
-    int dcount = 0;
-    unsigned sparity = 0;
-    for (int i = gt; i < 2 * kMaxDense * 2; i += kSegGroupThreads) c_acc[i] = 0.f;
-    named_bar_sync(1 + group, kSegGroupThreads);
-
-    for (unsigned seq = group;; seq += kSegGroups) {
-        const unsigned k = seq / kSegGroups;
-        const int stage = group * kSegDepth + (int)(k % kSegDepth);
-        mbar_wait_quiet(&full[stage], (k / kSegDepth) & 1u);
-        const SegDesc* d = &desc[stage];
-        const int kind = d->kind;
-        if (kind < 0) break;
-        const int64_t plane = d->plane;
-        const int chunk = d->chunk;
-        const int warp_vecs = (kind == 2 ? p.apply_elems : kSegItemElems) / 4 / kSegGroupWarps;
-        const int wvec = min(max(d->nvec - gw * warp_vecs, 0), warp_vecs);
-        const int64_t sample = (int)plane / (int)p.channels;
-        unsigned char* st = stages + (size_t)stage * STAGE_BYTES;
-        const float4* a4 = reinterpret_cast<const float4*>(st) + gw * warp_vecs;
-        const float4* b4 = reinterpret_cast<const float4*>(st + kSegHalfElems * 4) + gw * warp_vecs;
-        const uint32_t* l4 = reinterpret_cast<const uint32_t*>(st + kSegDataBytes) + gw * warp_vecs;
-
-        {
-            if (sample != cached_sample) {
-                named_bar_sync(1 + group, kSegGroupThreads);
-                for (int l = gt; l < kLabels; l += kSegGroupThreads) c_dense[l] = __ldg(p.dense + sample * kLabels + l);
-                dcount = __ldg(p.dense_count + sample);
-                named_bar_sync(1 + group, kSegGroupThreads);
-                cached_sample = sample;
+    const float* cbase = p.content + src_plane(p.cmap, plane) * p.hw_c;
+    const float* pbase = PREV ? p.prev + plane * p.hw_c : nullptr;
+    float* obase = p.out + sample * p.out_batch_stride + (plane - sample * p.channels) * p.hw_c;
+    const uint32_t* lbase = reinterpret_cast<const uint32_t*>(p.c_lab + sample * p.hw_c);
+    const int64_t nvec = p.hw_c / 4;
+    for (int ch = c0; ch < c1; ++ch) {
+        float4 v[U], q[U];
+        uint32_t lw[U];
+#pragma unroll
+        for (int u = 0; u < U; ++u) {
+            const int64_t idx = ((int64_t)ch * U + u) * kSegApplyThreads + threadIdx.x;
+            if (idx < nvec) {
+                v[u] = ldg_f4_hint(cbase + idx * 4, pol_first);
+                if (PREV) q[u] = ldg_f4_hint(pbase + idx * 4, pol_first);
+                lw[u] = __ldg(lbase + idx);
             }
         }
-
-        if (kind <= 1) {
-            const int64_t key = plane * 2 + kind;
-            if (key != cached_stat) {
-                named_bar_sync(1 + group, kSegGroupThreads);
-                for (int l = gt; l < kLabels; l += kSegGroupThreads) c_shift[l] = __ldg(p.shift + key * kLabels + l);
-                named_bar_sync(1 + group, kSegGroupThreads);
-                cached_stat = key;
-            }
-            float* acc = c_acc + sparity * (kMaxDense * 2);
-            int cur = -1;
-            uint32_t cur4 = 0xffffffffu;
-            float shift = 0.f, a1 = 0.f, a2 = 0.f;
-            float4 vv[kSegLaneVecs];
-            uint32_t lww[kSegLaneVecs];
-#pragma unroll
-            for (int j = 0; j < kSegLaneVecs; ++j) {
-                const int idx = lane * kSegLaneVecs + ((j + lane) & (kSegLaneVecs - 1));
-                if (idx < wvec) { vv[j] = a4[idx]; lww[j] = l4[idx]; }
-            }
-            __syncwarp();
-            if (lane == 0) mbar_arrive(&empty[stage]);
-#pragma unroll
-            for (int j = 0; j < kSegLaneVecs; ++j) {
-                const int idx = lane * kSegLaneVecs + ((j + lane) & (kSegLaneVecs - 1));
-                if (idx < wvec) {
-                    const float4 v = vv[j];
-                    const uint32_t lw = lww[j];
-                    if (lw == cur4 && cur >= 0) {
-                        const float d0 = v.x - shift, d1 = v.y - shift, d2 = v.z - shift, d3 = v.w - shift;
-                        a1 += (d0 + d1) + (d2 + d3);
-                        a2 = fmaf(d0, d0, a2); a2 = fmaf(d1, d1, a2); a2 = fmaf(d2, d2, a2); a2 = fmaf(d3, d3, a2);
-                    } else {
-                        const float e[4] = {v.x, v.y, v.z, v.w};
-                        int curl = cur >= 0 ? (int)(cur4 & 0xffu) : -1;
-#pragma unroll
-                        for (int q = 0; q < 4; ++q) {
-                            const int l = (int)((lw >> (8 * q)) & 0xffu);
-                            if (l != curl) {
-                                if (cur >= 0) {
-                                    atomicAdd(&acc[cur * 2 + 0], a1);
-                                    atomicAdd(&acc[cur * 2 + 1], a2);
-                                }
-                                const int dn = c_dense[l];
-                                curl = l;
-                                if (dn != 255) { cur = dn; shift = c_shift[l]; cur4 = (uint32_t)l * 0x01010101u; }
-                                else { cur = -1; cur4 = 0xffffffffu; }
-                                a1 = 0.f; a2 = 0.f;
-                            }
-                            if (cur >= 0) {
-                                const float dd = e[q] - shift;
-                                a1 += dd;
-                                a2 = fmaf(dd, dd, a2);
-                            }
-                        }
-                    }
+#pragma unroll
+        for (int u = 0; u < U; ++u) {
+            const int64_t idx = ((int64_t)ch * U + u) * kSegApplyThreads + threadIdx.x;
+            if (idx < nvec) {
+                const uint32_t b0 = lw[u] & 0xffu;
+                float4 o;
+                if (lw[u] == b0 * 0x01010101u) {
+                    const float4 cf = s_coef[b0];
+                    o.x = fmaf(v[u].x - cf.x, cf.y, cf.z);
+                    o.y = fmaf(v[u].y - cf.x, cf.y, cf.z);
+                    o.z = fmaf(v[u].z - cf.x, cf.y, cf.z);
+                    o.w = fmaf(v[u].w - cf.x, cf.y, cf.z);
+                } else {
+                    const float4 k0 = s_coef[b0], k1 = s_coef[(lw[u] >> 8) & 0xffu], k2 = s_coef[(lw[u] >> 16) & 0xffu],
+                                 k3 = s_coef[lw[u] >> 24];
+                    o.x = fmaf(v[u].x - k0.x, k0.y, k0.z);
+                    o.y = fmaf(v[u].y - k1.x, k1.y, k1.z);
+                    o.z = fmaf(v[u].z - k2.x, k2.y, k2.z);
+                    o.w = fmaf(v[u].w - k3.x, k3.y, k3.z);
                 }
-            }
-            const bool staged = dcount <= 32;
-            float* wt = c_wtot + (sparity * kSegGroupWarps + gw) * 64;
-            if (staged) {
-                seg_warp_totals(reinterpret_cast<float2*>(wt), lane, cur, a1, a2);
-            } else if (cur >= 0) {
-                atomicAdd(&acc[cur * 2 + 0], a1);
-                atomicAdd(&acc[cur * 2 + 1], a2);
-            }
-            named_bar_sync(1 + group, kSegGroupThreads);
-            if (gt < dcount) {
-                float t1 = acc[gt * 2 + 0], t2 = acc[gt * 2 + 1];
-                if (staged) {
-                    const float* w0 = c_wtot + sparity * kSegGroupWarps * 64;
-#pragma unroll
-                    for (int q = 0; q < kSegGroupWarps; ++q) { t1 += w0[q * 64 + gt * 2 + 0]; t2 += w0[q * 64 + gt * 2 + 1]; }
-                }
-                const float s1 = canon_f(t1), s2 = canon_f(t2);
-                acc[gt * 2 + 0] = 0.f;
-                acc[gt * 2 + 1] = 0.f;
-                float2* slot = p.slots + ((key * p.imax + chunk) * kMaxDense + gt);
-                asm volatile("st.global.cg.v2.f32 [%0], {%1,%2};" :: "l"(slot), "f"(s1), "f"(s2) : "memory");
-            }
-            sparity ^= 1u;
-        } else if (kind == 2) {
-            if (plane != cached_apply) {
-                if (lane == 0 && ld_acquire(&p.ready[plane]) == 0) {
-                    const uint64_t t0 = global_timer_ns();
-                    while (ld_acquire(&p.ready[plane]) == 0) {
-                        __nanosleep(64);
-                        if (watchdog_expired(t0)) __trap();
-                    }
-                }
-                named_bar_sync(1 + group, kSegGroupThreads);
-                if (gt < dcount) c_coef[gt] = __ldcg(&p.coef[plane * kLabels + __ldg(p.label_of + sample * kMaxDense + gt)]);
-                if (gt == kSegGroupThreads - 1) c_coef[kMaxDense] = make_float4(0.f, 1.f, 0.f, 0.f);
-                named_bar_sync(1 + group, kSegGroupThreads);
-                cached_apply = plane;
-            }
-            const bool has_prev = p.prev != nullptr;
-            float4* o4 = reinterpret_cast<float4*>(p.out + sample * p.out_batch_stride + (plane - sample * p.channels) * p.hw_c +
-                                                   (int64_t)chunk * p.apply_elems) + gw * warp_vecs;
-            uint32_t last_w = 0;
-            float4 cf = c_coef[kMaxDense];
-            bool have = false;
-            auto coef_of = [&](uint32_t l) -> float4 { const int dn = c_dense[l]; return c_coef[dn < kMaxDense ? dn : kMaxDense]; };
-#pragma unroll 8
-            for (int j = 0; j < kSegLaneVecs; ++j) {
-                const int idx = j * 32 + lane;
-                if (idx < wvec) {
-                    const float4 v = a4[idx];
-                    const uint32_t lw = l4[idx];
-                    float4 o;
-                    const uint32_t b0 = lw & 0xffu;
-                    if (lw == b0 * 0x01010101u) {
-                        if (!have || lw != last_w) { cf = coef_of(b0); last_w = lw; have = true; }
-                        o.x = fmaf(v.x - cf.x, cf.y, cf.z);
-                        o.y = fmaf(v.y - cf.x, cf.y, cf.z);
-                        o.z = fmaf(v.z - cf.x, cf.y, cf.z);
-                        o.w = fmaf(v.w - cf.x, cf.y, cf.z);
-                    } else {
-                        const float4 c0 = coef_of(b0), c1 = coef_of((lw >> 8) & 0xffu), c2 = coef_of((lw >> 16) & 0xffu),
-                                     c3 = coef_of(lw >> 24);
-                        o.x = fmaf(v.x - c0.x, c0.y, c0.z);
-                        o.y = fmaf(v.y - c1.x, c1.y, c1.z);
-                        o.z = fmaf(v.z - c2.x, c2.y, c2.z);
-                        o.w = fmaf(v.w - c3.x, c3.y, c3.z);
-                    }
-                    if (has_prev) {
-                        const float4 q = b4[idx];
-                        o.x += q.x; o.y += q.y; o.z += q.z; o.w += q.w;
-                    }
-                    stg_f4_hint(reinterpret_cast<float*>(o4 + idx), o, pol_first);
-                }
-            }
-            __syncwarp();
-            if (lane == 0) mbar_arrive(&empty[stage]);
+                if (PREV) { o.x += q[u].x; o.y += q[u].y; o.z += q[u].z; o.w += q[u].w; }
+                stg_f4_hint(obase + idx * 4, o, pol_first);
+            }
         }
     }
 }
@@ -877,20 +656,28 @@
 
 inline bool aligned(const void* p, size_t a) { return (reinterpret_cast<uintptr_t>(p) & (a - 1)) == 0; }
 
+void seg_plan_schedule(SegTmaParams& q, bool has_prev) {
+    q.ic = (int)((q.hw_c + kSegItemElems - 1) / kSegItemElems);
+    q.is = (int)((q.hw_s + kSegItemElems - 1) / kSegItemElems);
+    q.apply_elems = has_prev ? kSegPrevElems : kSegItemElems;
+    q.ia = (int)((q.hw_c + q.apply_elems - 1) / q.apply_elems);
+    q.row_items = (int)g_knobs.seg_stats_items;
+    q.rc = (q.ic + q.row_items - 1) / q.row_items;
+    q.rs = (q.is + q.row_items - 1) / q.row_items;
+}
+
 struct SegTmaLayout {
-    size_t ticket, zero_beg, ready, cnt, dcount, overflow, zero_end, first, first_bytes, shift, dense, label_of, coef,
-        slots, slots_bytes, total;
+    size_t zero_beg, cnt, dcount, overflow, zero_end, first, first_bytes, shift, dense, label_of, coef, rows, total;
 };
 SegTmaLayout seg_tma_layout(int64_t n, int64_t c, int64_t hw_c, int64_t hw_s) {
     const size_t planes = (size_t)(n * c);
-    const size_t ic = (size_t)((hw_c + kSegItemElems - 1) / kSegItemElems), is = (size_t)((hw_s + kSegItemElems - 1) / kSegItemElems);
-    const size_t imax = ic > is ? ic : is;
+    SegTmaParams q{};
+    q.hw_c = hw_c; q.hw_s = hw_s;
+    seg_plan_schedule(q, false);
     SegTmaLayout l;
     size_t o = 0;
     auto take = [&](size_t bytes) { size_t at = o; o += align_up(bytes, 256); return at; };
-    l.ticket = take(256);
     l.zero_beg = o;
-    l.ready = take(planes * sizeof(int));
     l.cnt = take((size_t)n * 2 * kLabels * sizeof(int));
     l.dcount = take((size_t)n * sizeof(int));
     l.overflow = take(sizeof(int));
@@ -901,28 +688,29 @@
     l.dense = take((size_t)n * kLabels);
     l.label_of = take((size_t)n * kMaxDense);
     l.coef = take(planes * kLabels * sizeof(float4));
-    l.slots_bytes = planes * 2 * imax * kMaxDense * sizeof(float2);
-    l.slots = take(l.slots_bytes);
+    l.rows = take(planes * (size_t)(q.rc + q.rs) * kMaxDense * sizeof(double2));
     l.total = o;
     return l;
 }
 
-int launch_seg_tma(const SegTmaParams& p, cudaStream_t st) {
-    constexpr size_t stage = kSegStageBytes;
-    constexpr size_t cache = kSegCacheBytes;
-    constexpr size_t smem = kSegGroups * (kSegDepth * stage + cache) + kSegGroups * kSegDepth * sizeof(SegDesc) +
-                            2 * kSegGroups * kSegDepth * sizeof(uint64_t) + 2 * kSegMailbox * sizeof(uint64_t) +
-                            kSegMailbox * sizeof(int64_t) +
-                            kSegTicketBatch * sizeof(SegDecoded);
+int launch_seg_split(const SegTmaParams& p, cudaStream_t st) {
     static PerDeviceFlag configured_on;
     bool& configured = configured_on.get();
     if (!configured) {
-        RPST_CUDA(cudaFuncSetAttribute(seg_tma_kernel, cudaFuncAttributeMaxDynamicSharedMemorySize, (int)smem));
+        RPST_CUDA(cudaFuncSetAttribute(seg_stats_kernel, cudaFuncAttributePreferredSharedMemoryCarveout,
+                                       (int)cudaSharedmemCarveoutMaxShared));
         configured = true;
     }
-    int64_t grid = sm_count();
-    if (grid > (int64_t)p.total_items) grid = p.total_items;
-    seg_tma_kernel<<<(int)grid, 32 + kSegGroups * kSegGroupThreads + kSegMergeThreads, smem, st>>>(p);
+    const int64_t planes = p.n * p.channels;
+    const int64_t stat_ctas = planes * (p.rc + p.rs);
+    const int64_t apply_ctas = planes * ((p.ia + kSegApplyChunks - 1) / kSegApplyChunks);
+    RPST_CHECK_ARG(stat_ctas < (1ll << 31) && apply_ctas < (1ll << 31), "seg_adain: too many work items; split the call");
+    seg_stats_kernel<<<(unsigned)stat_ctas, 32 + kSegGroupThreads, 0, st>>>(p);
+    RPST_CUDA(cudaGetLastError());
+    seg_merge_kernel<<<(unsigned)planes, kMaxDense, 0, st>>>(p);
+    RPST_CUDA(cudaGetLastError());
+    if (p.prev) seg_apply_kernel<true><<<(unsigned)apply_ctas, kSegApplyThreads, 0, st>>>(p);
+    else seg_apply_kernel<false><<<(unsigned)apply_ctas, kSegApplyThreads, 0, st>>>(p);
     RPST_CUDA(cudaGetLastError());
     return RPST_OK;
 }
@@ -932,29 +720,26 @@
 
 namespace rpst {
 namespace {
-int64_t seg_plan_schedule(SegTmaParams& q, bool has_prev) {
-    const int64_t planes = q.n * q.channels;
-    q.ic = (int)((q.hw_c + kSegItemElems - 1) / kSegItemElems);
-    q.is = (int)((q.hw_s + kSegItemElems - 1) / kSegItemElems);
-    q.imax = q.ic > q.is ? q.ic : q.is;
-    q.apply_elems = has_prev ? kSegPrevElems : kSegItemElems;
-    q.ia = (int)((q.hw_c + q.apply_elems - 1) / q.apply_elems);
-    const int64_t plane_bytes = q.hw_c * (int64_t)sizeof(float);
-    int64_t lag = (g_knobs.seg_lag_bytes + plane_bytes - 1) / plane_bytes;
-    if (lag < 3) lag = 3;
-    q.lag = (int)(lag < planes ? lag : planes);
-    return planes * ((int64_t)q.ic + q.is + 1 + q.ia);
-}
-
-__global__ void seg_schedule_dump_kernel(SegTmaParams p, int32_t* out) {
-    const unsigned t = blockIdx.x * blockDim.x + threadIdx.x;
-    if (t >= p.total_items) return;
-    int kind = -1, chunk = 0;
-    int64_t plane = 0;
-    seg_decode(t, p, kind, plane, chunk);
-    out[3 * (size_t)t + 0] = kind;
-    out[3 * (size_t)t + 1] = (int32_t)plane;
-    out[3 * (size_t)t + 2] = chunk;
+__global__ void seg_schedule_dump_kernel(SegTmaParams p, int64_t total, int32_t* out) {
+    const int64_t t = blockIdx.x * (int64_t)blockDim.x + threadIdx.x;
+    if (t >= total) return;
+    const int64_t planes = p.n * p.channels, st = p.ic + p.is;
+    int kind, chunk;
+    int64_t plane;
+    if (t < planes * st) {
+        plane = t / st;
+        const int u = (int)(t % st);
+        kind = u < p.ic ? 0 : 1;
+        chunk = u < p.ic ? u : u - p.ic;
+    } else if (t < planes * (st + 1)) {
+        kind = 3; plane = t - planes * st; chunk = 0;
+    } else {
+        const int64_t a = t - planes * (st + 1);
+        kind = 2; plane = a / p.ia; chunk = (int)(a % p.ia);
+    }
+    out[3 * t + 0] = kind;
+    out[3 * t + 1] = (int32_t)plane;
+    out[3 * t + 2] = chunk;
 }
 }
 }
@@ -967,13 +752,13 @@
     RPST_CHECK_ARG(n > 0 && c > 0 && hw_c > 0 && hw_s > 0 && info != nullptr, "debug_seg_schedule: bad arguments");
     SegTmaParams q{};
     q.n = n; q.channels = c; q.hw_c = hw_c; q.hw_s = hw_s;
-    const int64_t total = seg_plan_schedule(q, has_prev != 0);
+    seg_plan_schedule(q, has_prev != 0);
+    const int64_t planes = n * c, total = planes * ((int64_t)q.ic + q.is + 1 + q.ia);
     RPST_CHECK_ARG(total < (1ll << 31), "debug_seg_schedule: too many tickets");
-    q.total_items = (unsigned)total;
-    info[0] = total; info[1] = q.ic; info[2] = q.is; info[3] = q.ia; info[4] = q.lag;
+    info[0] = total; info[1] = q.ic; info[2] = q.is; info[3] = q.ia; info[4] = planes;
     if (tickets != nullptr) {
         RPST_CHECK_ARG(max_tickets >= total, "debug_seg_schedule: ticket buffer too small");
-        seg_schedule_dump_kernel<<<(unsigned)((total + 255) / 256), 256, 0, static_cast<cudaStream_t>(stream)>>>(q, tickets);
+        seg_schedule_dump_kernel<<<(unsigned)((total + 255) / 256), 256, 0, static_cast<cudaStream_t>(stream)>>>(q, total, tickets);
         RPST_CUDA(cudaGetLastError());
     }
     return RPST_OK;
@@ -1045,8 +830,6 @@
         q.content = content; q.style = style; q.c_lab = c_labels; q.s_lab = s_labels; q.prev = prev; q.out = out;
         q.cmap = content_map; q.smap = style_map;
         q.n = n; q.channels = c; q.hw_c = hw_c; q.hw_s = hw_s; q.out_batch_stride = out_batch_stride; q.eps = eps;
-        q.ticket = reinterpret_cast<unsigned*>(base + t.ticket);
-        q.ready = reinterpret_cast<int*>(base + t.ready);
         int* cnt = reinterpret_cast<int*>(base + t.cnt);
         int* first = reinterpret_cast<int*>(base + t.first);
         int* dcount = reinterpret_cast<int*>(base + t.dcount);
@@ -1056,11 +839,9 @@
         q.cnt = cnt; q.first = first; q.dense = dense; q.label_of = label_of; q.dense_count = dcount; q.overflow = overflow;
         q.shift = reinterpret_cast<float*>(base + t.shift);
         q.coef = reinterpret_cast<float4*>(base + t.coef);
-        q.slots = reinterpret_cast<float2*>(base + t.slots);
-        RPST_CUDA(cudaMemsetAsync(base + t.ticket, 0xff, 256, st));
+        q.rows = reinterpret_cast<double2*>(base + t.rows);
         RPST_CUDA(cudaMemsetAsync(base + t.zero_beg, 0, t.zero_end - t.zero_beg, st));
         RPST_CUDA(cudaMemsetAsync(base + t.first, 0x7f, t.first_bytes, st));
-        RPST_CUDA(cudaMemsetAsync(base + t.slots, 0xff, t.slots_bytes, st));
         seg_hist_kernel<<<dim3(hist_blocks0, (unsigned)n, 2), 256, 0, st>>>(c_labels, s_labels, hw_c, hw_s, cnt, first);
         RPST_CUDA(cudaGetLastError());
         seg_dense_kernel<<<(unsigned)n, kLabels, 0, st>>>(cnt, dense, label_of, dcount, overflow);
@@ -1074,10 +855,8 @@
         const int64_t planes = n * c;
         seg_shift_kernel<<<(unsigned)((planes * 2 * kLabels + 255) / 256), 256, 0, st>>>(q);
         RPST_CUDA(cudaGetLastError());
-        const int64_t total = seg_plan_schedule(q, prev != nullptr);
-        RPST_CHECK_ARG(total < (1ll << 31), "seg_adain: too many work items (%lld); split the call", (long long)total);
-        q.total_items = (unsigned)total;
-        const int rc = launch_seg_tma(q, st);
+        seg_plan_schedule(q, prev != nullptr);
+        const int rc = launch_seg_split(q, st);
         if (rc) return rc;
         run_flag = overflow;
         base += t.total;
diff --git a/rp-style-transfer_b200/csrc/tuning.cuh b/rp-style-transfer_b200/csrc/tuning.cuh
--- a/rp-style-transfer_b200/csrc/tuning.cuh
+++ b/rp-style-transfer_b200/csrc/tuning.cuh
@@ -12,7 +12,7 @@
     int64_t adain_twin_apply = 1;
     int64_t adain_group_merge_min_spp = 512;
     int64_t adain_merge_lead = 0;
-    int64_t seg_lag_bytes = 256ll << 20;
+    int64_t seg_stats_items = 16;
     int64_t attn_flash = 1;
     int64_t attn_flash_prof = 0;
     int64_t wct_fused_cov = 1;
```

Result: no change. 3487, median of 6 (+0.3%).
